# ruotianluo/ImageCaptioning.pytorch

Hardware: NVIDIA H100
Metric: captions/sec at beam=5 seq_len=20 (higher is better)
Workload: dtype f32 (fp32-grade: split-fp16 x3 tensor-core passes, fp32 accumulate)

## Files before the change

imagecaptioning.pytorch_b200/_lib.py:

```python
from __future__ import annotations

import ctypes
import os
from ctypes import POINTER, Structure, c_char_p, c_double, c_float, c_int, c_long, c_longlong, c_ulonglong, c_void_p

PKG = os.path.dirname(os.path.abspath(__file__))
LIB_PATH = os.path.join(PKG, 'libcapb200.so')

MODE_SIMT_FP32, MODE_TC_F16X3, MODE_TC_F16X1 = 0, 1, 2
MODES = {'simt_fp32': MODE_SIMT_FP32, 'tc_f16x3': MODE_TC_F16X3, 'tc_f16x1': MODE_TC_F16X1}
OP_MODES = dict(MODES, skinny_tf32x3=3, skinny_fp32=4, tf32x3_tc=5, tf32x3_tc_dgrad=6, tf32x3_tc_wgrad=7)
FAMILY_UPDOWN, FAMILY_NEWFC, FAMILY_ATT2IN2 = 0, 1, 2
FAMILY_AOA = 3
ENSEMBLE_MAX_MEMBERS = 8
SAMPLE_GREEDY, SAMPLE_MULTINOMIAL, SAMPLE_FORCED, SAMPLE_TEACHER, SAMPLE_TOPK, SAMPLE_TOPP = 0, 1, 2, 3, 4, 5


class ModelCfg(Structure):
    _fields_ = [('family', c_int), ('vocab_size', c_int), ('input_encoding_size', c_int), ('rnn_size', c_int), ('att_hid_size', c_int),
                ('fc_feat_size', c_int), ('att_feat_size', c_int), ('seq_length', c_int), ('numeric_mode', c_int)]


WEIGHT_FIELDS = ['embed', 'fc_embed_w', 'fc_embed_b', 'att_embed_w', 'att_embed_b', 'ctx2att_w', 'ctx2att_b', 'logit_w', 'logit_b',
                 'att_lstm_w_ih', 'att_lstm_w_hh', 'att_lstm_b_ih', 'att_lstm_b_hh', 'lang_lstm_w_ih', 'lang_lstm_w_hh', 'lang_lstm_b_ih',
# ... 107 lines not shown


class MhaWeights(Structure):
    _fields_ = [(f, c_void_p) for f in ('q_w', 'q_b', 'k_w', 'k_b', 'v_w', 'v_b', 'o_w', 'o_b')]


class TfmEncLayer(Structure):
    _fields_ = [('self_attn', MhaWeights)] + [(f, c_void_p) for f in ('w1_w', 'w1_b', 'w2_w', 'w2_b', 'ln0_a', 'ln0_b', 'ln1_a', 'ln1_b')]


class TfmDecLayer(Structure):
    _fields_ = [('self_attn', MhaWeights), ('src_attn', MhaWeights)] + \
               [(f, c_void_p) for f in ('w1_w', 'w1_b', 'w2_w', 'w2_b', 'ln0_a', 'ln0_b', 'ln1_a', 'ln1_b', 'ln2_a', 'ln2_b')]


class TfmWeights(Structure):
    _fields_ = [('att_embed_w', c_void_p), ('att_embed_b', c_void_p), ('enc', TfmEncLayer * TFM_MAX_LAYERS), ('enc_norm_a', c_void_p),
                ('enc_norm_b', c_void_p), ('dec', TfmDecLayer * TFM_MAX_LAYERS), ('dec_norm_a', c_void_p), ('dec_norm_b', c_void_p),
                ('lut', c_void_p), ('pe', c_void_p), ('gen_w', c_void_p), ('gen_b', c_void_p)]


class TfmXeOpts(Structure):
    _fields_ = [('seq_per_img', c_int), ('seed', c_ulonglong), ('label_smoothing', c_float), ('upstream', c_float), ('drop_prob_lm', c_float),
                ('dropout', c_float), ('att_masks', c_void_p), ('keep_rows', c_int), ('row_loss', c_void_p)]


class TfmScstOpts(Structure):
    _fields_ = [('sample_n', c_int), ('temperature', c_float), ('seed', c_ulonglong), ('upstream', c_float), ('baseline', c_int),
                ('drop_prob_lm', c_float), ('dropout', c_float), ('forced_tokens', c_void_p), ('att_masks', c_void_p), ('keep_rows', c_int),
                ('row_loss', c_void_p), ('sampler', POINTER(SamplerOpts)), ('reward_weights', POINTER(RewardWeights))]


class VjpOpts(Structure):
    _fields_ = [('forward_only', c_int), ('dlogprobs', c_void_p), ('greedy', c_int)]


AOA_REFINER_LAYERS = 6


class AoaCfg(Structure):
    _fields_ = [(f, c_int) for f in ('vocab_size', 'input_encoding_size', 'rnn_size', 'heads', 'att_feat_size', 'seq_length', 'numeric_mode')]


class AoaRefinerLayer(Structure):
    _fields_ = [(f, c_void_p) for f in ('q_w', 'q_b', 'k_w', 'k_b', 'v_w', 'v_b', 'aoa_w', 'aoa_b', 'ln_a', 'ln_b')]


class AoaWeights(Structure):
    _fields_ = [('embed', c_void_p), ('att_embed_w', c_void_p), ('att_embed_b', c_void_p), ('refiner', AoaRefinerLayer * AOA_REFINER_LAYERS)] + \
               [(f, c_void_p) for f in ('refiner_norm_a', 'refiner_norm_b', 'ctx2att_w', 'ctx2att_b', 'att_lstm_w_ih', 'att_lstm_w_hh', 'att_lstm_b_ih',
                                        'att_lstm_b_hh', 'attn_norm_a', 'attn_norm_b', 'attn_q_w', 'attn_q_b', 'att2ctx_w', 'att2ctx_b', 'logit_w',
                                        'logit_b')]


class GemmEpilogue(Structure):
    _fields_ = [('bias', c_void_p), ('row_bias', c_void_p), ('ld_row_bias', c_long), ('rows_per_group', c_int), ('residual', c_void_p),
                ('ld_res', c_long), ('relu', c_int), ('C', c_void_p), ('ldc', c_long), ('C_hi', c_void_p), ('C_lo', c_void_p), ('ldcs', c_long),
                ('lstm', c_int), ('H', c_int), ('c_prev', c_void_p), ('ld_cprev', c_long), ('src_row', c_void_p), ('c_out', c_void_p),
                ('ld_cout', c_long), ('gather_bias', c_void_p), ('ld_gb', c_long), ('gather_idx', c_void_p), ('h_f', c_void_p), ('h_hi', c_void_p),
                ('h_lo', c_void_p), ('ld_h', c_long)]


SIGNATURES = {
    'capb200_last_error': (c_char_p, []),
    'capb200_abi_version': (c_int, []),
    'capb200_range_status': (c_int, [c_int]),
    'capb200_linear': (c_int, [c_void_p, c_long, c_void_p, c_long, c_void_p, c_void_p, c_long, c_int, c_int, c_int, c_int, c_int, c_void_p]),
    'capb200_bench_linear': (c_int, [c_void_p, c_void_p, c_void_p, c_void_p, c_int, c_int, c_int, c_int, c_int, c_void_p, c_void_p]),
    'capb200_gemm_tile_n': (c_int, [c_int, c_int]),
    'capb200_gemm_tile_m': (c_int, [c_int, c_int]),
    'capb200_lstm_cell': (c_int, [c_void_p, c_int, c_void_p, c_void_p, c_void_p, c_void_p, c_void_p, c_void_p, c_void_p, c_void_p, c_int, c_int,
                                  c_int, c_void_p]),
    'capb200_additive_attention': (c_int, [c_void_p, c_void_p, c_void_p, c_void_p, c_void_p, c_void_p, c_void_p, c_int, c_int, c_int, c_int, c_int,
                                           c_void_p]),
    'capb200_log_softmax_topk': (c_int, [c_void_p, c_long, c_int, c_int, c_int, c_int, c_void_p, c_void_p, c_void_p]),
    'capb200_vocab_stats_topk': (c_int, [c_void_p, c_long, c_int, c_int, c_int, c_int, c_void_p, c_void_p, c_void_p, c_void_p]),
    'capb200_vocab_select': (c_int, [c_void_p, c_long, c_int, c_int, c_int, c_float, c_float, c_ulonglong, c_ulonglong, c_void_p, c_int, c_void_p,
                                     c_void_p, c_void_p]),
    'capb200_engine_create': (c_void_p, [POINTER(ModelCfg)]),
    'capb200_engine_destroy': (None, [c_void_p]),
    'capb200_engine_bind_weights': (c_int, [c_void_p, POINTER(Weights), c_void_p]),
    'capb200_decode_beam': (c_int, [c_void_p, c_void_p, c_void_p, c_void_p, c_int, c_int, POINTER(BeamOpts), c_void_p, c_void_p, c_void_p, c_void_p,
                                    c_void_p, c_void_p, c_void_p]),
    'capb200_beam_record_logprobs': (c_int, [c_void_p, c_int, c_int, c_void_p, c_void_p]),
    'capb200_decode_beam_diverse': (c_int, [c_void_p, c_void_p, c_void_p, c_void_p, c_int, c_int, POINTER(DiverseOpts), c_void_p, c_void_p, c_void_p,
                                            c_void_p, c_void_p, c_void_p, c_void_p]),
    'capb200_decode_sample': (c_int, [c_void_p, c_void_p, c_void_p, c_void_p, c_int, c_int, POINTER(SampleOpts), c_void_p, c_long, c_void_p, c_void_p,
                                      c_void_p, c_void_p]),
    'capb200_engine_launch_count': (c_long, [c_void_p]),
    'capb200_engine_set_profiling': (c_int, [c_void_p, c_int]),
    'capb200_engine_read_profile': (c_int, [c_void_p, c_int, c_void_p, c_void_p, c_void_p, c_int]),
    'capb200_tfm_create': (c_void_p, [POINTER(TfmCfg)]),
    'capb200_tfm_destroy': (None, [c_void_p]),
    'capb200_tfm_bind_weights': (c_int, [c_void_p, POINTER(TfmWeights), c_void_p]),
    'capb200_tfm_decode_beam': (c_int, [c_void_p, c_void_p, c_void_p, c_int, c_int, POINTER(BeamOpts), c_void_p, c_void_p, c_void_p, c_void_p, c_void_p,
                                        c_void_p, c_void_p]),
    'capb200_tfm_beam_record_logprobs': (c_int, [c_void_p, c_int, c_int, c_void_p, c_void_p]),
    'capb200_tfm_decode_sample': (c_int, [c_void_p, c_void_p, c_void_p, c_int, c_int, POINTER(SampleOpts), c_void_p, c_long, c_void_p, c_void_p, c_void_p,
                                          c_void_p]),
    'capb200_tfm_launch_count': (c_long, [c_void_p]),
    'capb200_aoa_create': (c_void_p, [POINTER(AoaCfg)]),
    'capb200_aoa_destroy': (None, [c_void_p]),
    'capb200_aoa_bind_weights': (c_int, [c_void_p, POINTER(AoaWeights), c_void_p]),
    'capb200_aoa_decode_beam': (c_int, [c_void_p, c_void_p, c_void_p, c_int, c_int, POINTER(BeamOpts), c_void_p, c_void_p, c_void_p, c_void_p, c_void_p,
                                        c_void_p, c_void_p]),
    'capb200_aoa_beam_record_logprobs': (c_int, [c_void_p, c_int, c_int, c_void_p, c_void_p]),
    'capb200_aoa_decode_beam_diverse': (c_int, [c_void_p, c_void_p, c_void_p, c_int, c_int, POINTER(DiverseOpts), c_void_p, c_void_p, c_void_p, c_void_p,
                                                c_void_p, c_void_p, c_void_p]),
    'capb200_aoa_decode_sample': (c_int, [c_void_p, c_void_p, c_void_p, c_int, c_int, POINTER(SampleOpts), c_void_p, c_long, c_void_p, c_void_p, c_void_p,
                                          c_void_p]),
    'capb200_aoa_scst_step': (c_int, [c_void_p, c_void_p, c_int, c_int, POINTER(AoaScstOpts), c_void_p, c_void_p, c_void_p, c_int, POINTER(AoaWeights),
                                      c_void_p, c_void_p, c_void_p, c_void_p, c_void_p, c_void_p]),
    'capb200_aoa_xe_step': (c_int, [c_void_p, c_void_p, c_int, c_int, POINTER(AoaXeOpts), c_void_p, c_void_p, c_int, POINTER(AoaWeights), c_void_p,
                                    c_void_p, c_void_p]),
    'capb200_aoa_launch_count': (c_long, [c_void_p]),
    'capb200_ensemble_create': (c_void_p, []),
    'capb200_ensemble_destroy': (None, [c_void_p]),
    'capb200_ensemble_decode_beam': (c_int, [c_void_p, c_void_p, c_int, c_void_p, c_void_p, c_void_p, c_int, c_int, POINTER(BeamOpts), c_void_p, c_void_p,
                                             c_void_p, c_void_p, c_void_p, c_void_p, c_void_p]),
    'capb200_ensemble_beam_record_logprobs': (c_int, [c_void_p, c_int, c_int, c_void_p, c_void_p]),
    'capb200_ensemble_decode_sample': (c_int, [c_void_p, c_void_p, c_int, c_void_p, c_void_p, c_void_p, c_int, c_int, POINTER(SampleOpts), c_void_p, c_long,
                                               c_void_p, c_void_p, c_void_p, c_void_p]),
    'capb200_ensemble_launch_count': (c_long, [c_void_p]),
    'capb200_updown_scst_step': (c_int, [c_void_p, c_void_p, c_void_p, c_int, c_int, POINTER(ScstOpts), c_void_p, c_void_p, c_void_p, c_int,
                                         POINTER(UpdownGrads), c_void_p, c_void_p, c_void_p, c_void_p, c_void_p, c_void_p]),
    'capb200_att2in2_scst_step': (c_int, [c_void_p, c_void_p, c_void_p, c_int, c_int, POINTER(ScstOpts), c_void_p, c_void_p, c_void_p, c_int,
                                          POINTER(Att2in2Grads), c_void_p, c_void_p, c_void_p, c_void_p, c_void_p, c_void_p]),
    'capb200_att2in2_xe_step': (c_int, [c_void_p, c_void_p, c_void_p, c_int, c_int, POINTER(XeOpts), c_void_p, c_void_p, c_int, POINTER(Att2in2Grads),
                                        c_void_p, c_void_p, c_void_p]),
    'capb200_newfc_scst_step': (c_int, [c_void_p, c_void_p, c_void_p, c_int, c_int, POINTER(ScstOpts), c_void_p, c_void_p, c_void_p, c_int,
                                        POINTER(NewfcGrads), c_void_p, c_void_p, c_void_p, c_void_p, c_void_p, c_void_p]),
    'capb200_newfc_xe_step': (c_int, [c_void_p, c_void_p, c_void_p, c_int, c_int, POINTER(XeOpts), c_void_p, c_void_p, c_int, POINTER(NewfcGrads),
                                      c_void_p, c_void_p, c_void_p]),
    'capb200_dropout_mask': (c_int, [c_void_p, c_long, c_ulonglong, c_int, c_int, c_float, c_void_p]),
    'capb200_mha_forward': (c_int, [c_int, c_int, c_int, c_int, c_int, c_int, c_void_p, c_void_p, c_void_p, c_long, c_void_p, c_long, c_ulonglong, c_int,
                                    c_float, c_void_p, c_long, c_void_p]),
    'capb200_mha_self_backward': (c_int, [c_int, c_int, c_int, c_int, c_int, c_void_p, c_void_p, c_void_p, c_long, c_void_p, c_long, c_ulonglong, c_int,
                                          c_float, c_void_p, c_long, c_void_p, c_void_p, c_void_p, c_long, c_void_p]),
    'capb200_mha_cross_backward': (c_int, [c_int, c_int, c_int, c_int, c_int, c_int, c_int, c_void_p, c_long, c_void_p, c_void_p, c_long, c_ulonglong,
                                           c_int, c_int, c_float, c_void_p, c_void_p, c_long, c_void_p, c_long, c_void_p, c_void_p, c_long, c_void_p]),
    'capb200_mha_causal_forward': (c_int, [c_int, c_int, c_int, c_int, c_int, c_int, c_int, c_void_p, c_void_p, c_void_p, c_long, c_void_p, c_long,
                                           c_ulonglong, c_int, c_float, c_void_p, c_long, c_void_p]),
    'capb200_mha_causal_backward': (c_int, [c_int, c_int, c_int, c_int, c_int, c_void_p, c_void_p, c_void_p, c_long, c_void_p, c_long, c_ulonglong,
                                            c_int, c_float, c_void_p, c_long, c_void_p, c_void_p, c_void_p, c_long, c_void_p]),
    'capb200_tfm_dec_self_attention': (c_int, [c_int, c_int, c_int, c_int, c_int, c_void_p, c_long, c_void_p, c_void_p, c_long, c_long, c_void_p,
                                               c_long, c_void_p, c_long, c_void_p, c_long, c_void_p]),
    'capb200_tfm_xe_step': (c_int, [c_void_p, c_void_p, c_int, c_int, POINTER(TfmXeOpts), c_void_p, c_void_p, c_int, POINTER(TfmWeights), c_void_p, c_void_p,
                                    c_void_p]),
    'capb200_tfm_scst_step': (c_int, [c_void_p, c_void_p, c_int, c_int, POINTER(TfmScstOpts), c_void_p, c_void_p, c_void_p, c_int, POINTER(TfmWeights),
                                      c_void_p, c_void_p, c_void_p, c_void_p, c_void_p, c_void_p]),
    'capb200_tfm_set_grad_events': (c_int, [c_void_p, c_void_p, c_int]),
    'capb200_adam_chunk_elems': (c_int, []),
    'capb200_adam_step': (c_int, [c_void_p, c_void_p, c_void_p, c_int, c_double, c_double, c_double, c_double, c_double, c_long, c_double, c_int, c_void_p]),
    'capb200_engine_set_grad_events': (c_int, [c_void_p, c_void_p, c_int]),
    'capb200_aoa_set_grad_events': (c_int, [c_void_p, c_void_p, c_int]),
    'capb200_cider_table_create': (c_void_p, [c_void_p, c_void_p, c_long, c_double, c_void_p]),
    'capb200_cider_table_destroy': (None, [c_void_p]),
    'capb200_cider_corpus_table_create': (c_void_p, []),
    'capb200_cider_table_reserve': (c_int, [c_void_p, c_long, c_int]),
    'capb200_cider_table_is_corpus': (c_int, [c_void_p]),
    'capb200_cider_scores': (c_int, [c_void_p, c_void_p, c_int, c_int, c_int, c_void_p, c_void_p, c_int, c_void_p, c_void_p, c_void_p]),
    'capb200_bleu4_scores': (c_int, [c_void_p, c_int, c_void_p, c_int, c_int, c_void_p, c_void_p, c_int, c_void_p, c_void_p]),
    'capb200_weighted_reward': (c_int, [c_void_p, POINTER(RewardWeights), c_void_p, c_int, c_void_p, c_int, c_int, c_void_p, c_void_p, c_int, c_void_p,
                                        c_void_p, c_void_p, c_void_p]),
    'capb200_updown_xe_step': (c_int, [c_void_p, c_void_p, c_void_p, c_int, c_int, POINTER(XeOpts), c_void_p, c_void_p, c_int, c_void_p, c_void_p,
                                       c_void_p, c_void_p]),
# ... 68 lines not shown
```

imagecaptioning.pytorch_b200/csrc/beam.cu:

```cuda
#include "../../include/capb200.h"
#include "common.cuh"
#include "kernels.cuh"

namespace capb200 {

namespace {

constexpr int MAXB = 16;

__device__ __forceinline__ double apply_penalty(int kind, float alpha, int length, double p) {
    if (kind == 1) return p / (pow(5.0 + length, (double)alpha) / pow(6.0, (double)alpha));
    if (kind == 2) return p / (double)length;
    return p;
}

__device__ __forceinline__ void select_step(const BeamState& s, int img, int t, int live, int kl, int row0, int hist0, const float* __restrict__ top_val,
                                            const int* __restrict__ top_idx, const int* pen, int n_pen, float lambda, int penalty_kind,
                                            float penalty_alpha, double* __restrict__ done_p) {
    const int lane = threadIdx.x;
    const int b = s.beam, T = s.T;
    const int ncand = live * kl;
    float cv[8];
    int cf[8];
#pragma unroll
    for (int u = 0; u < 8; ++u) {
        const int c = lane + 32 * u;
        cv[u] = -INFINITY;
        cf[u] = 0x7fffffff;
        if (c < ncand) {
            const int pb = c / kl, k = c % kl;
            const long row = (long)row0 + pb;
            const int w = top_idx[row * kl + k];
            float v = top_val[row * kl + k];
            int cnt = 0;
            for (int q = 0; q < n_pen; ++q) cnt += (pen[q] == w);
            if (cnt) v = __fsub_rn(v, __fmul_rn((float)cnt, lambda));
            cv[u] = s.sums[(long)img * b + pb] + v;
            cf[u] = pb * s.V1 + w;
        }
    }
    const int* seq_old = (t & 1) ? s.seq_b : s.seq_a;
    int* seq_new = (t & 1) ? s.seq_a : s.seq_b;
    const int* hist_old = (t & 1) ? s.hist_b : s.hist_a;
    int* hist_new = (t & 1) ? s.hist_a : s.hist_b;

    float my_v = -INFINITY;
    int my_f = 0;
    for (int j = 0; j < b; ++j) {
        float bv = -INFINITY;
        int bf = 0x7fffffff, bu = -1;
#pragma unroll
        for (int u = 0; u < 8; ++u)
            if (cv[u] > bv || (cv[u] == bv && cf[u] < bf)) { bv = cv[u]; bf = cf[u]; bu = u; }
        float wv = bv;
        int wf = bf;
#pragma unroll
        for (int o = 16; o > 0; o >>= 1) {
            const float ov = __shfl_xor_sync(0xffffffffu, wv, o);
            const int of = __shfl_xor_sync(0xffffffffu, wf, o);
            if (ov > wv || (ov == wv && of < wf)) { wv = ov; wf = of; }
        }
        if (bu >= 0 && bf == wf && bv == wv) {
#pragma unroll
            for (int u = 0; u < 8; ++u) if (u == bu) { cv[u] = -INFINITY; cf[u] = 0x7fffffff; }
        }
        if (lane == j) { my_v = wv; my_f = wf; }
    }
    __shared__ int sh_parent[MAXB], sh_word[MAXB], sh_slot[MAXB];
    const bool has = lane < b;
    const int parent = has ? my_f / s.V1 : 0;
    const int word = has ? my_f % s.V1 : 0;
    const bool ended = has && ((word == 0) || (t == T - 1));
    const unsigned em = __ballot_sync(0xffffffffu, ended);
    const int cnt0 = s.done_cnt[img];
    const int slot = cnt0 + __popc(em & ((1u << lane) - 1u));
    if (has) { sh_parent[lane] = parent; sh_word[lane] = word; sh_slot[lane] = ended ? slot : -1; }
    __syncwarp();
    for (int idx = lane; idx < b * t; idx += 32) {
        const int j = idx / t, q = idx - j * t;
        const long dst = ((long)img * b + j) * T, src = ((long)img * b + sh_parent[j]) * T;
        seq_new[dst + q] = seq_old[src + q];
        hist_new[dst + q] = hist_old[src + q];
    }
    if (em != 0u) {
        for (int idx = lane; idx < b * (t + 1); idx += 32) {
            const int j = idx / (t + 1), q = idx - j * (t + 1);
            if (sh_slot[j] < 0) continue;
            const long rec = ((long)img * b * T + sh_slot[j]) * T, src = ((long)img * b + sh_parent[j]) * T;
            s.done_seq[rec + q] = (q < t) ? seq_old[src + q] : sh_word[j];
            s.done_hist[rec + q] = (q < t) ? hist_old[src + q] : hist0 + sh_parent[j];
        }
    }
    if (has) {
        const long dst = ((long)img * b + lane) * T;
        seq_new[dst + t] = word;
        hist_new[dst + t] = hist0 + parent;
        float new_sum = my_v;
        if (ended) {
            const long rec = (long)img * b * T + slot;
            s.done_len[rec] = t + 1;
            s.done_raw[rec] = new_sum;
            done_p[rec] = apply_penalty(penalty_kind, penalty_alpha, t + 1, (double)new_sum);
            new_sum -= 1000.0f;
        }
        s.sums[(long)img * b + lane] = new_sum;
        s.tokens[(long)img * b + lane] = word;
        s.src_row[(long)img * b + lane] = row0 + parent;
    }
    if (lane == 0 && em != 0u) s.done_cnt[img] = cnt0 + __popc(em);
}

__global__ void __launch_bounds__(32) beam_step_kernel(BeamState s, int t, int live, const float* __restrict__ top_val,
                                                       const int* __restrict__ top_idx, int penalty_kind, float penalty_alpha,
                                                       double* __restrict__ done_p) {
    const int img = blockIdx.x;
    select_step(s, img, t, live, s.beam, img * live, img * live, top_val, top_idx, nullptr, 0, 0.f, penalty_kind, penalty_alpha, done_p);
}

__global__ void __launch_bounds__(32) diverse_beam_step_kernel(BeamState s, int G, int t, int k, const float* __restrict__ top_val,
                                                               const int* __restrict__ top_idx, float lambda, int rows_total, int penalty_kind,
                                                               float penalty_alpha, double* __restrict__ done_p) {
    const int i = blockIdx.x, lane = threadIdx.x;
    const int b = s.beam, T = s.T;
    __shared__ int sh_pen[MAXB];
    for (int g = 0; g < G && g <= t; ++g) {
        const int lt = t - g;
        if (lt >= T) continue;
        const int n_pen = g * b;
        __syncwarp();
        if (lane < n_pen) {
            const int pg = lane / b, j = lane - pg * b;
            const int last = min(t - pg, T - 1);
            const int* seq_pg = (last & 1) ? s.seq_a : s.seq_b;
            sh_pen[lane] = seq_pg[((long)(i * G + pg) * b + j) * T + lt];
        }
        __syncwarp();
        const int vimg = i * G + g;
        select_step(s, vimg, lt, lt == 0 ? 1 : b, k, vimg * b, g * rows_total + vimg * b, top_val, top_idx, sh_pen, n_pen, lambda, penalty_kind,
                    penalty_alpha, done_p);
    }
}

__global__ void __launch_bounds__(32) beam_finalize_kernel(BeamState s, int keep, const double* __restrict__ done_p, long long* __restrict__ out_seq,
                                                           int* __restrict__ out_len, float* __restrict__ out_p, float* __restrict__ out_raw,
                                                           int* __restrict__ out_hist) {
    const int img = blockIdx.x, lane = threadIdx.x;
    const int b = s.beam, T = s.T;
    const int cnt = s.done_cnt[img];
    const long base = (long)img * b * T;
    extern __shared__ unsigned char taken[];
    for (int i = lane; i < cnt; i += 32) taken[i] = 0;
    __syncwarp();
    for (int k = 0; k < keep; ++k) {
        double bv = -INFINITY;
        int bi = 0x7fffffff;
        for (int i = lane; i < cnt; i += 32) {
            if (!taken[i]) {
                const double v = done_p[base + i];
                if (v > bv || (v == bv && i < bi)) { bv = v; bi = i; }
            }
        }
#pragma unroll
        for (int o = 16; o > 0; o >>= 1) {
            const double ov = __shfl_xor_sync(0xffffffffu, bv, o);
            const int oi = __shfl_xor_sync(0xffffffffu, bi, o);
            if (ov > bv || (ov == bv && oi < bi)) { bv = ov; bi = oi; }
        }
        const long o = (long)img * keep + k;
        if (bi == 0x7fffffff) {
            if (lane == 0) { out_len[o] = 0; out_p[o] = -INFINITY; out_raw[o] = -INFINITY; }
            for (int q = lane; q < T; q += 32) { out_seq[o * T + q] = 0; out_hist[o * T + q] = -1; }
            continue;
        }
        if (lane == 0) {
            taken[bi] = 1;
            out_len[o] = s.done_len[base + bi];
            out_p[o] = (float)bv;
            out_raw[o] = s.done_raw[base + bi];
        }
        const int len = s.done_len[base + bi];
        for (int q = lane; q < T; q += 32) {
            out_seq[o * T + q] = (q < len) ? (long long)s.done_seq[(base + bi) * T + q] : 0;
            out_hist[o * T + q] = (q < len) ? s.done_hist[(base + bi) * T + q] : -1;
        }
        __syncwarp();
    }
}

__global__ void beam_edit_kernel(int rows, int k_in, int beam, int t, DecodeEdits ed, const int* __restrict__ prev_tokens,
                                 const float* __restrict__ val_in, const int* __restrict__ idx_in, float* __restrict__ val_out, int* __restrict__ idx_out,
                                 int first_beam, int first_group_rows, int first_group) {
    const int r = blockIdx.x * blockDim.x + threadIdx.x;
    if (r >= rows) return;
    if (first_beam > 0 && (r % first_beam) / first_group_rows == first_group) t = 0;
    float v[MAXB];
    int ix[MAXB];
    const int prev = (t > 0 && prev_tokens != nullptr) ? prev_tokens[r] : -1;
    bool prev_bad = false;
    if (t > 0 && ed.n_bad > 0)
        for (int i = 0; i < ed.n_bad; ++i) prev_bad |= (ed.bad[i] == prev);
    for (int k = 0; k < k_in; ++k) {
        float x = val_in[(long)r * k_in + k];
        const int w = idx_in[(long)r * k_in + k];
        if (ed.constraint && t > 0 && w == prev) x = -INFINITY;
        if (prev_bad && w == 0) x = -INFINITY;
        if (w == ed.unk_col) x -= 1000.0f;
        v[k] = x;
        ix[k] = w;
    }
    for (int j = 0; j < beam; ++j) {
        int best = j;
        for (int k = j + 1; k < k_in; ++k)
            if (v[k] > v[best] || (v[k] == v[best] && ix[k] < ix[best])) best = k;
        const float tv = v[j]; v[j] = v[best]; v[best] = tv;
        const int ti = ix[j]; ix[j] = ix[best]; ix[best] = ti;
        val_out[(long)r * beam + j] = v[j];
        idx_out[(long)r * beam + j] = ix[j];
    }
}

__global__ void scale_rows_kernel(float* __restrict__ x, long ld, int rows, int cols, float f, int skip_beam, int skip_group_rows, int skip_group) {
    const long total = (long)rows * cols;
// ... 16 lines not shown
        return;
    }
    auto apply_edits = [&]() {
        if (seqs == nullptr || !ed.any()) return;
        __syncthreads();
        if (threadIdx.x == 0) {
            const int prev = sidx > 0 ? (int)seqs[item - 1] : -1;
            if (ed.unk_col >= 0 && ed.unk_col < V1) d[ed.unk_col] -= 1000.0f;
            if (ed.constraint && prev >= 0 && prev < V1) d[prev] = -INFINITY;
            bool prev_bad = false;
            for (int i = 0; i < ed.n_bad; ++i) prev_bad |= (sidx > 0 && ed.bad[i] == prev);
            if (prev_bad) d[0] = -INFINITY;
        }
    };
    const float* src = slab + (long)sidx * step_stride + (long)row * ld_slab;
    if (stats != nullptr) {
        const float2 st = stats[(long)sidx * stats_stride + row];
        const float mx = st.x, lsum = st.y;
        const float m2 = (mx - mx) - lsum, l2 = lsum;
        const bool twice = sidx > 0;
        const bool vec4 = ((V1 & 3) == 0) && ((ld_slab & 3) == 0) && ((step_stride & 3) == 0) && ((reinterpret_cast<uintptr_t>(slab) & 15) == 0) &&
                          ((reinterpret_cast<uintptr_t>(dst) & 15) == 0);
        if (vec4) {
            const float4* s4 = reinterpret_cast<const float4*>(src);
            float4* d4 = reinterpret_cast<float4*>(d);
            for (int v = threadIdx.x; v < V1 / 4; v += blockDim.x) {
                const float4 x = __ldg(s4 + v);
                float4 o;
                o.x = (x.x - mx) - lsum; o.y = (x.y - mx) - lsum; o.z = (x.z - mx) - lsum; o.w = (x.w - mx) - lsum;
                if (twice) { o.x = (o.x - m2) - l2; o.y = (o.y - m2) - l2; o.z = (o.z - m2) - l2; o.w = (o.w - m2) - l2; }
                d4[v] = o;
            }
        } else {
            for (int v = threadIdx.x; v < V1; v += blockDim.x) {
                const float lp = (src[v] - mx) - lsum;
                d[v] = twice ? (lp - m2) - l2 : lp;
            }
        }
        apply_edits();
        return;
    }
    const bool vec = ((V1 & 3) == 0) && ((ld_slab & 3) == 0) && ((step_stride & 3) == 0) && ((reinterpret_cast<uintptr_t>(slab) & 15) == 0) &&
                     ((reinterpret_cast<uintptr_t>(dst) & 15) == 0);
    if (vec) {
        const float4* s4 = reinterpret_cast<const float4*>(src);
        float4* d4 = reinterpret_cast<float4*>(d);
        for (int v = threadIdx.x; v < V1 / 4; v += blockDim.x) d4[v] = __ldg(s4 + v);
    } else {
        for (int v = threadIdx.x; v < V1; v += blockDim.x) d[v] = src[v];
    }
    apply_edits();
}

}

int beam_edit_launch(int rows, int k_in, int beam, int t, const DecodeEdits& ed, const int* prev_tokens, const float* val_in, const int* idx_in,
                     float* val_out, int* idx_out, cudaStream_t stream, int first_beam, int first_group_rows, int first_group) {
    CAPB_REQUIRE(k_in >= beam && k_in <= MAXB, "beam_size + number of active decode edits must be <= 16");
    if (rows <= 0) return 0;
    beam_edit_kernel<<<cdiv(rows, 128), 128, 0, stream>>>(rows, k_in, beam, t, ed, prev_tokens, val_in, idx_in, val_out, idx_out, first_beam,
                                                          first_group_rows, first_group);
    CAPB_CHECK_CUDA(cudaGetLastError());
    return 0;
}

int scale_rows_launch(float* x, long ld, int rows, int cols, float factor, cudaStream_t stream, int skip_beam, int skip_group_rows, int skip_group) {
    if (rows <= 0 || cols <= 0) return 0;
    long blocks = ((long)rows * cols + 255) / 256;
    if (blocks > sm_count() * 16) blocks = sm_count() * 16;
    scale_rows_kernel<<<(int)blocks, 256, 0, stream>>>(x, ld, rows, cols, factor, skip_beam, skip_group_rows, skip_group);
    CAPB_CHECK_CUDA(cudaGetLastError());
    return 0;
}

int beam_step_launch(const BeamState& s, int t, int live, const float* top_val, const int* top_idx, int penalty_kind, float penalty_alpha,
                     cudaStream_t stream) {
    CAPB_REQUIRE(s.beam >= 1 && s.beam <= MAXB, "beam size 1..16");
    CAPB_REQUIRE(s.beam * s.T <= MAXB * CAPB200_MAX_SEQ_LENGTH, "beam*T record capacity (16 x CAPB200_MAX_SEQ_LENGTH)");
    beam_step_kernel<<<s.B, 32, 0, stream>>>(s, t, live, top_val, top_idx, penalty_kind, penalty_alpha, s.done_p);
    CAPB_CHECK_CUDA(cudaGetLastError());
    return 0;
}

int diverse_beam_step_launch(const BeamState& s, int G, int t, int k, const float* top_val, const int* top_idx, float lambda, int rows_total,
                             int penalty_kind, float penalty_alpha, cudaStream_t stream) {
    CAPB_REQUIRE(G >= 2 && s.beam >= 1 && G * s.beam <= MAXB, "group_size * beams per group must be in 2..16");
    CAPB_REQUIRE(k >= s.beam && k <= MAXB && s.beam * k <= 256, "candidate list width");
    CAPB_REQUIRE(s.beam * s.T <= MAXB * CAPB200_MAX_SEQ_LENGTH, "beam*T record capacity (16 x CAPB200_MAX_SEQ_LENGTH)");
    CAPB_REQUIRE(lambda >= 0.f, "diversity_lambda must be >= 0 (the candidate lists rely on the penalty only lowering values)");
    diverse_beam_step_kernel<<<s.B / G, 32, 0, stream>>>(s, G, t, k, top_val, top_idx, lambda, rows_total, penalty_kind, penalty_alpha, s.done_p);
    CAPB_CHECK_CUDA(cudaGetLastError());
    return 0;
}

int beam_finalize_launch(const BeamState& s, int keep, long long* out_seq, int* out_len, float* out_p, float* out_raw, int* out_hist,
                         cudaStream_t stream) {
    CAPB_REQUIRE(keep >= 1 && keep <= s.beam, "keep must be in 1..beam");
    beam_finalize_kernel<<<s.B, 32, (size_t)s.beam * s.T, stream>>>(s, keep, s.done_p, out_seq, out_len, out_p, out_raw, out_hist);
    CAPB_CHECK_CUDA(cudaGetLastError());
    return 0;
}

int gather_logprob_rows_launch(const float* slab, long step_stride, long ld_slab, const int* hist, int nseq, int T, int V1, float* dst,
                               const float2* stats, long stats_stride, cudaStream_t stream, const long long* seqs, const DecodeEdits* ed) {
    if (nseq <= 0) return 0;
    gather_rows_kernel<<<nseq * T, 256, 0, stream>>>(slab, step_stride, ld_slab, hist, T, V1, dst, stats, stats_stride, seqs, ed ? *ed : DecodeEdits());
    CAPB_CHECK_CUDA(cudaGetLastError());
    return 0;
}

}
```

imagecaptioning.pytorch_b200/csrc/engine.cu:

```cuda
#include <map>
#include <mutex>
#include <vector>

#include "../../include/capb200.h"
#include "common.cuh"
#include "kernels.cuh"
#include "engine_common.cuh"
#include "train_common.cuh"

namespace capb200 {

static thread_local std::string g_last_error;
void set_error(const std::string& msg) { g_last_error = msg; }
const char* last_error_cstr() { return g_last_error.c_str(); }

__global__ void capb_fill_int_kernel(int* p, int n, int v) {
    const int i = blockIdx.x * blockDim.x + threadIdx.x;
    if (i < n) p[i] = v;
}
__global__ void capb_load_token_column_kernel(const long long* src, long ld, int col, int n, int* dst) {
    const int i = blockIdx.x * blockDim.x + threadIdx.x;
    if (i < n) dst[i] = (int)src[(long)i * ld + col];
}
__global__ void capb_store_token_column_kernel(const int* src, int n, long long* dst, long ld, int col) {
// ... 218 lines not shown
    }
    return gemm_tc_plan_launch(e->plans[id], &g.epi, g.M, st);
}

int run_gemm(capb200_engine* e, int id, GemmProblem& g, int plan_rows, cudaStream_t st) {
    if (!e->profiling) return run_gemm_inner(e, id, g, plan_rows, st);
    if (e->ev_used + 2 > e->ev_pool.size()) {
        for (int i = 0; i < 64; ++i) {
            cudaEvent_t ev;
            CAPB_CHECK_CUDA(cudaEventCreate(&ev));
            e->ev_pool.push_back(ev);
        }
    }
    double k_total = 0;
    for (int s = 0; s < g.nseg; ++s) k_total += g.seg[s].K;
    CAPB_CHECK_CUDA(cudaEventRecord(e->ev_pool[e->ev_used], st));
    const int rc = run_gemm_inner(e, id, g, plan_rows, st);
    CAPB_CHECK_CUDA(cudaEventRecord(e->ev_pool[e->ev_used + 1], st));
    e->ev_used += 2;
    e->ev_ids.push_back(id);
    e->ev_flops.push_back(2.0 * g.M * g.N * k_total);
    return rc;
}

int prepare(capb200_engine* e, const float* fc, const float* att, const float* mask, int B, int R, cudaStream_t st) {
    CAPB_NVTX("capb200 prepare_feature (fc_embed, att_embed, ctx2att)");
    const int H = e->H, E = e->E, A = e->A;
    const bool updown = e->cfg.family == CAPB200_FAMILY_UPDOWN;
    const capb200_weights& w = e->w;
    ActView fc_in;  fc_in.f = const_cast<float*>(fc);  fc_in.ld = e->cfg.fc_feat_size;
    if (e->tc && e->cfg.family != CAPB200_FAMILY_ATT2IN2) {
        e->launches++;
        if (split_planes_launch(fc, e->cfg.fc_feat_size, B, e->cfg.fc_feat_size, e->in_fc.hi, e->in_fc.lo, e->in_fc.ld, st)) return 1;
    }
    if (e->cfg.family != CAPB200_FAMILY_ATT2IN2) {
        GemmProblem g;
        g.M = B; g.N = updown ? H : E; g.nseg = 1;
        g.seg[0] = seg_of(fc_in, w.fc_embed_w, e->cfg.fc_feat_size, e->p_fc, e->cfg.fc_feat_size);
        g.seg[0].A_hi = e->in_fc.hi; g.seg[0].A_lo = e->in_fc.lo; g.seg[0].lda_h = e->in_fc.ld;
        g.epi.bias = w.fc_embed_b; g.epi.relu = updown ? 1 : 0;
        g.epi.C = e->fc_e.v.f; g.epi.ldc = e->fc_e.v.ld; g.epi.C_hi = e->fc_e.v.hi; g.epi.C_lo = e->fc_e.v.lo; g.epi.ldcs = e->fc_e.v.ld;
        if (run_gemm(e, G_FC, g, e->capB, st)) return 1;
    }
    if (!attends(e)) return 0;
    ActView att_in; att_in.f = const_cast<float*>(att); att_in.ld = e->cfg.att_feat_size;
    if (e->tc) {
        e->launches++;
        if (split_planes_launch(att, e->cfg.att_feat_size, B * R, e->cfg.att_feat_size, e->in_att.hi, e->in_att.lo, e->in_att.ld, st)) return 1;
    }
    {
        GemmProblem g;
        g.M = B * R; g.N = H; g.nseg = 1;
        g.seg[0] = seg_of(att_in, w.att_embed_w, e->cfg.att_feat_size, e->p_attw, e->cfg.att_feat_size);
        g.seg[0].A_hi = e->in_att.hi; g.seg[0].A_lo = e->in_att.lo; g.seg[0].lda_h = e->in_att.ld;
        g.epi.bias = w.att_embed_b; g.epi.relu = 1;
        g.epi.C = e->att_e.v.f; g.epi.ldc = e->att_e.v.ld; g.epi.C_hi = e->att_e.v.hi; g.epi.C_lo = e->att_e.v.lo; g.epi.ldcs = e->att_e.v.ld;
        if (run_gemm(e, G_ATT, g, e->capB * e->capR, st)) return 1;
    }
    if (mask != nullptr) {
        e->launches++;
        if (mask_rows_launch(e->att_e.v, B, R, H, mask, R, st)) return 1;
    }
    {
        GemmProblem g;
        g.M = B * R; g.N = A; g.nseg = 1;
        g.seg[0] = seg_of(e->att_e.v, w.ctx2att_w, H, e->p_ctx, H);
        g.epi.bias = w.ctx2att_b;
        g.epi.C = e->p_att.v.f; g.epi.ldc = e->p_att.v.ld;
        if (run_gemm(e, G_CTX, g, e->capB * e->capR, st)) return 1;
    }
    if (!updown) return 0;
    {
        GemmProblem g;
        g.M = B; g.N = 4 * H; g.nseg = 1;
        g.seg[0] = seg_of(e->fc_e.v, w.att_lstm_w_ih + H, E + 2 * H, e->p_a_ih_fc, H);
        g.epi.bias = e->tc ? e->bsum_att_il : e->bsum_att;
        g.epi.C = e->g_fc.v.f; g.epi.ldc = e->g_fc.v.ld;
        if (run_gemm(e, G_GFC, g, e->capB, st)) return 1;
    }
    return 0;
}

int core_step(capb200_engine* e, int rows, int rpi, const int* tokens, const int* src_row, float* logits, long ld_logits, int n_images, int R,
              const float* mask, cudaStream_t st) {
    const int H = e->H, E = e->E, A = e->A, V1 = e->V1;
    const capb200_weights& w = e->w;
    if (e->cfg.family == CAPB200_FAMILY_UPDOWN) {
        StateCopy s0, s1;
        s0.src = e->h0_out.v.f; s0.ld_src = e->h0_out.v.ld; s0.dst = e->h0_in.v;
        s1.src = e->h1_out.v.f; s1.ld_src = e->h1_out.v.ld; s1.dst = e->h1_in.v;
        const bool xg = e->use_xgate;
        e->launches++;
        if (state_gather_embed_launch(rows, tokens, src_row, w.embed, E, xg ? 0 : E, 1, e->xt.v, H, 2, s0, s1, st)) return 1;
        const int cur = e->core_cur, nxt = cur ^ 1;
        {
            GemmProblem g;
            g.M = rows; g.N = 4 * H;
            g.seg[0] = seg_of(e->h1_in.v, w.att_lstm_w_ih, E + 2 * H, e->p_a_ih_h, H);
            g.seg[1] = seg_of(e->h0_in.v, w.att_lstm_w_hh, H, e->p_a_hh, H);
            g.nseg = 2;
            if (!xg) { g.seg[2] = seg_of(e->xt.v, w.att_lstm_w_ih + 2 * H, E + 2 * H, e->p_a_ih_x, E); g.nseg = 3; }
            g.epi.row_bias = e->g_fc.v.f; g.epi.ld_row_bias = e->g_fc.v.ld; g.epi.rows_per_group = rpi;
            if (e->tc) {
                g.epi.lstm = 1; g.epi.H = H;
                g.epi.c_prev = e->c0[cur]; g.epi.ld_cprev = e->ld_c; g.epi.src_row = src_row;
                g.epi.c_out = e->c0[nxt]; g.epi.ld_cout = e->ld_c;
                g.epi.gather_bias = xg ? e->xgate : nullptr; g.epi.ld_gb = e->ld_xgate; g.epi.gather_idx = tokens;
                g.epi.h_f = e->h0_out.v.f; g.epi.h_hi = e->h0_out.v.hi; g.epi.h_lo = e->h0_out.v.lo; g.epi.ld_h = e->h0_out.v.ld;
            } else {
                g.epi.C = e->gates.v.f; g.epi.ldc = e->gates.v.ld;
            }
            if (run_gemm(e, G_LSTM1, g, e->capRows, st)) return 1;
        }
        if (!e->tc) {
            e->launches++;
            if (lstm_pointwise_launch(rows, H, e->gates.v.f, e->gates.v.ld, src_row, e->c0[cur], e->ld_c, e->c0[nxt], e->ld_c, e->h0_out.v,
                                      xg ? e->xgate : nullptr, e->ld_xgate, tokens, st)) return 1;
        }
        {
            GemmProblem g;
            g.M = rows; g.N = A; g.nseg = 1;
            g.seg[0] = seg_of(e->h0_out.v, w.h2att_w, H, e->p_h2att, H);
            g.epi.bias = w.h2att_b;
            g.epi.C = e->att_h.v.f; g.epi.ldc = e->att_h.v.ld;
            if (run_gemm(e, G_H2ATT, g, e->capRows, st)) return 1;
        }
        e->launches += 2;
        if (additive_attention_launch(n_images, rpi, R, A, H, e->att_h.v.f, e->att_h.v.ld, e->p_att.v.f, e->p_att.v.ld, e->att_e.v.f, e->att_e.v.ld,
                                      mask, R, w.alpha_w, w.alpha_b, e->att_score, e->att_res.v, st)) return 1;
        {
            GemmProblem g;
            g.M = rows; g.N = 4 * H; g.nseg = 3;
            g.seg[0] = seg_of(e->att_res.v, w.lang_lstm_w_ih, 2 * H, e->p_l_ih_a, H);
            g.seg[1] = seg_of(e->h0_out.v, w.lang_lstm_w_ih + H, 2 * H, e->p_l_ih_h, H);
            g.seg[2] = seg_of(e->h1_in.v, w.lang_lstm_w_hh, H, e->p_l_hh, H);
            if (e->tc) {
                g.epi.bias = e->bsum_lang_il;
                g.epi.lstm = 1; g.epi.H = H;
                g.epi.c_prev = e->c1[cur]; g.epi.ld_cprev = e->ld_c; g.epi.src_row = src_row;
                g.epi.c_out = e->c1[nxt]; g.epi.ld_cout = e->ld_c;
                g.epi.h_f = e->h1_out.v.f; g.epi.h_hi = e->h1_out.v.hi; g.epi.h_lo = e->h1_out.v.lo; g.epi.ld_h = e->h1_out.v.ld;
            } else {
                g.epi.bias = e->bsum_lang;
                g.epi.C = e->gates.v.f; g.epi.ldc = e->gates.v.ld;
            }
            if (run_gemm(e, G_LSTM2, g, e->capRows, st)) return 1;
        }
        if (!e->tc) {
            e->launches++;
            if (lstm_pointwise_launch(rows, H, e->gates.v.f, e->gates.v.ld, src_row, e->c1[cur], e->ld_c, e->c1[nxt], e->ld_c, e->h1_out.v,
                                      nullptr, 0, nullptr, st)) return 1;
        }
        e->core_cur = nxt;
        {
            GemmProblem g;
            g.M = rows; g.N = V1; g.nseg = 1;
            g.seg[0] = seg_of(e->h1_out.v, w.logit_w, H, e->p_logit, H);
            g.epi.bias = w.logit_b;
            g.epi.C = logits; g.epi.ldc = ld_logits;
            if (run_gemm(e, G_LOGIT, g, e->capRows, st)) return 1;
        }
        return 0;
    }
    if (e->cfg.family == CAPB200_FAMILY_ATT2IN2) {
        StateCopy s0, s1;
        s0.src = e->h0_out.v.f; s0.ld_src = e->h0_out.v.ld; s0.dst = e->h0_in.v;
        e->launches++;
        if (state_gather_embed_launch(rows, tokens, src_row, w.embed, E, E, 1, e->xt.v, H, 1, s0, s1, st)) return 1;
        const int cur = e->core_cur, nxt = cur ^ 1;
        {
            GemmProblem g;
            g.M = rows; g.N = A; g.nseg = 1;
            g.seg[0] = seg_of(e->h0_in.v, w.h2att_w, H, e->p_h2att, H);
            g.epi.bias = w.h2att_b;
            g.epi.C = e->att_h.v.f; g.epi.ldc = e->att_h.v.ld;
            if (run_gemm(e, G_H2ATT, g, e->capRows, st)) return 1;
// ... 16 lines not shown
            g.seg[0] = seg_of(e->att_res.v, w.a2c_w, H, e->p_a2c, H);
            g.epi.residual = e->gates.v.f + 3 * H; g.epi.ld_res = e->gates.v.ld;
            g.epi.C = e->gates.v.f + 3 * H; g.epi.ldc = e->gates.v.ld;
            if (run_gemm(e, G_A2C, g, e->capRows, st)) return 1;
        }
        e->launches++;
        if (maxout_pointwise_launch(rows, H, e->gates.v.f, e->gates.v.ld, src_row, e->c0[cur], e->ld_c, e->c0[nxt], e->ld_c, e->h0_out.v, st)) return 1;
        e->core_cur = nxt;
        GemmProblem g;
        g.M = rows; g.N = V1; g.nseg = 1;
        g.seg[0] = seg_of(e->h0_out.v, w.logit_w, H, e->p_logit, H);
        g.epi.bias = w.logit_b;
        g.epi.C = logits; g.epi.ldc = ld_logits;
        return run_gemm(e, G_LOGIT, g, e->capRows, st);
    }
    const bool fresh = (src_row == e->d.neg1);
    for (int pass = fresh ? 0 : 1; pass < 2; ++pass) {
        StateCopy s0, s1;
        s0.src = e->h0_out.v.f; s0.ld_src = e->h0_out.v.ld; s0.dst = e->h0_in.v;
        const int* srcs = (pass == 0) ? e->d.neg1 : (fresh ? nullptr : src_row);
        e->launches++;
        if (pass == 0) {
            if (state_gather_embed_launch(rows, e->img_of_row, srcs, e->fc_e.v.f, e->fc_e.v.ld, E, 0, e->xt.v, H, 1, s0, s1, st)) return 1;
        } else {
            if (state_gather_embed_launch(rows, tokens, srcs, w.embed, E, E, 0, e->xt.v, H, 1, s0, s1, st)) return 1;
        }
        const int cur = e->core_cur, nxt = cur ^ 1;
        GemmProblem g;
        g.M = rows; g.N = 5 * H; g.nseg = 2;
        g.seg[0] = seg_of(e->xt.v, w.i2h_w, E, e->p_i2h, E);
        g.seg[1] = seg_of(e->h0_in.v, w.h2h_w, H, e->p_h2h, H);
        g.epi.bias = e->bsum_core;
        g.epi.C = e->gates.v.f; g.epi.ldc = e->gates.v.ld;
        if (run_gemm(e, G_CORE, g, e->capRows, st)) return 1;
        e->launches++;
        if (maxout_pointwise_launch(rows, H, e->gates.v.f, e->gates.v.ld, srcs, e->c0[cur], e->ld_c, e->c0[nxt], e->ld_c, e->h0_out.v, st)) return 1;
        e->core_cur = nxt;
    }
    GemmProblem g;
    g.M = rows; g.N = V1; g.nseg = 1;
    g.seg[0] = seg_of(e->h0_out.v, w.logit_w, H, e->p_logit, H);
    g.epi.bias = w.logit_b;
    g.epi.C = logits; g.epi.ldc = ld_logits;
    return run_gemm(e, G_LOGIT, g, e->capRows, st);
}

int check_ready(capb200_engine* e) {
    CAPB_REQUIRE(e != nullptr, "null engine");
    CAPB_REQUIRE(e->bound, "capb200_engine_bind_weights has not been called");
    CAPB_CHECK_RANGE();
    return 0;
}

}

namespace capb200 {

int lstm_member_info(capb200_engine* e, MemberInfo* m) {
    if (check_ready(e)) return 1;
    m->family = e->cfg.family;
    m->V1 = e->V1; m->T = e->T;
    m->attends = attends(e);
    m->graph_ok = !e->profiling;
    m->ws = e->ws; m->wblock = e->wblock;
    m->fresh = e->d.neg1;
    m->launches = &e->launches;
    return 0;
}

int lstm_decode_workspace(capb200_engine* e, int B, int rows, int R, int beam, int rows_per_image, cudaStream_t st) {
    if (ensure_workspace(e, B, rows, R, beam, st)) return 1;
    if (!attends(e)) { iota_div_kernel<<<cdiv(rows, 256), 256, 0, st>>>(e->img_of_row, rows, rows_per_image); e->launches++; }
    return 0;
}

int lstm_decode_prepare(capb200_engine* e, const float* fc, const float* att, const float* mask, int B, int R, cudaStream_t st) {
    if (prepare(e, fc, att, mask, B, R, st)) return 1;
    e->core_cur = 0;
    return 0;
}

int lstm_decode_core(capb200_engine* e, int rows, int rpi, const int* tokens, const int* src_row, float* logits, long ld, int B, int R,
                     const float* mask, cudaStream_t st) {
    return core_step(e, rows, rpi, tokens, src_row, logits, ld, B, R, mask, st);
}

}

extern "C" {

const char* capb200_last_error(void) { return g_last_error.c_str(); }
int capb200_abi_version(void) { return CAPB200_ABI_VERSION; }
int capb200_range_status(int reset) { return range_flag_read(reset); }

capb200_engine* capb200_engine_create(const capb200_model_cfg* cfg) {
    if (cfg == nullptr) { set_error("null cfg"); return nullptr; }
    if (cfg->family != CAPB200_FAMILY_UPDOWN && cfg->family != CAPB200_FAMILY_NEWFC && cfg->family != CAPB200_FAMILY_ATT2IN2) {
        set_error("unknown model family");
        return nullptr;
    }
    if (cfg->numeric_mode < 0 || cfg->numeric_mode > 2) { set_error("unknown numeric mode"); return nullptr; }
    if (cfg->seq_length < 1 || cfg->seq_length > CAPB200_MAX_SEQ_LENGTH) { set_error("seq_length must be in 1..256 (CAPB200_MAX_SEQ_LENGTH)"); return nullptr; }
    int ndev = 0;
    if (cudaGetDeviceCount(&ndev) != cudaSuccess || ndev == 0) {
        set_error("no CUDA device: the capb200 engine has no CPU fallback");
        return nullptr;
    }
    capb200_engine* e = new capb200_engine();
    e->cfg = *cfg;
    e->V1 = cfg->vocab_size + 1;
    e->E = cfg->input_encoding_size;
    e->H = cfg->rnn_size;
    e->A = cfg->att_hid_size;
    e->T = cfg->seq_length;
    e->mode = cfg->numeric_mode;
    e->tc = cfg->numeric_mode != CAPB200_MODE_SIMT_FP32;
    return e;
}

void capb200_engine_destroy(capb200_engine* e) {
    if (e == nullptr) return;
    destroy_plans(e);
    for (cudaEvent_t ev : e->ev_pool) cudaEventDestroy(ev);
    cudaFree(e->wblock);
    cudaFree(e->ws);
    e->d.release();
    cudaFree(e->tape);
    e->sg.destroy();
    tf32_context_destroy(e->tf32);
    if (e->ev_gfork) cudaEventDestroy(e->ev_gfork);
    if (e->ev_gjoin) cudaEventDestroy(e->ev_gjoin);
    if (e->side) cudaStreamDestroy(e->side);
    delete e;
}

long capb200_engine_launch_count(const capb200_engine* e) { return e ? e->launches : 0; }

int capb200_engine_set_profiling(capb200_engine* e, int enable) {
    CAPB_REQUIRE(e != nullptr, "null engine");
    e->profiling = enable != 0;
    return 0;
}

int capb200_engine_read_profile(capb200_engine* e, int reset, double* ms, double* flops, long* calls, int n) {
    CAPB_REQUIRE(e != nullptr && n >= G_REPORTED, "need room for 9 GEMM ids");
    CAPB_CHECK_CUDA(cudaDeviceSynchronize());
    for (size_t i = 0; i < e->ev_ids.size(); ++i) {
        float t = 0.f;
        CAPB_CHECK_CUDA(cudaEventElapsedTime(&t, e->ev_pool[2 * i], e->ev_pool[2 * i + 1]));
        e->prof_ms[e->ev_ids[i]] += t;
        e->prof_flops[e->ev_ids[i]] += e->ev_flops[i];
        e->prof_calls[e->ev_ids[i]] += 1;
    }
    e->ev_ids.clear();
    e->ev_flops.clear();
    e->ev_used = 0;
    e->prof_ms[G_CORE] += e->prof_ms[G_A2C]; e->prof_flops[G_CORE] += e->prof_flops[G_A2C]; e->prof_calls[G_CORE] += e->prof_calls[G_A2C];
    e->prof_ms[G_A2C] = 0; e->prof_flops[G_A2C] = 0; e->prof_calls[G_A2C] = 0;
    for (int i = 0; i < G_REPORTED; ++i) {
        if (ms) ms[i] = e->prof_ms[i];
        if (flops) flops[i] = e->prof_flops[i];
        if (calls) calls[i] = e->prof_calls[i];
        if (reset) { e->prof_ms[i] = 0; e->prof_flops[i] = 0; e->prof_calls[i] = 0; }
    }
    return 0;
}

// ... 37 lines not shown
        if (att2in2) {
            add_vec_kernel<<<cdiv(2 * H, 256), 256, 0, st>>>(e->bsum_core + 3 * H, w->a2c_b, e->bsum_core + 3 * H, 2 * H);
            e->launches += 1;
        }
    }
    CAPB_CHECK_CUDA(cudaGetLastError());
    if (e->tc) {
        int rc = pack(e, w->logit_w, H, V1, H, e->p_logit, st);
        if (updown) {
            rc |= pack(e, w->fc_embed_w, e->cfg.fc_feat_size, H, e->cfg.fc_feat_size, e->p_fc, st);
            rc |= pack(e, w->att_embed_w, e->cfg.att_feat_size, H, e->cfg.att_feat_size, e->p_attw, st);
            rc |= pack(e, w->ctx2att_w, H, A, H, e->p_ctx, st);
            rc |= pack_gates(e, w->att_lstm_w_ih, E + 2 * H, H, H, e->p_a_ih_h, st);
            rc |= pack_gates(e, w->att_lstm_w_ih + H, E + 2 * H, H, H, e->p_a_ih_fc, st);
            rc |= pack_gates(e, w->att_lstm_w_ih + 2 * H, E + 2 * H, H, E, e->p_a_ih_x, st);
            rc |= pack_gates(e, w->att_lstm_w_hh, H, H, H, e->p_a_hh, st);
            rc |= pack_gates(e, w->lang_lstm_w_ih, 2 * H, H, H, e->p_l_ih_a, st);
            rc |= pack_gates(e, w->lang_lstm_w_ih + H, 2 * H, H, H, e->p_l_ih_h, st);
            rc |= pack_gates(e, w->lang_lstm_w_hh, H, H, H, e->p_l_hh, st);
            rc |= pack(e, w->h2att_w, H, A, H, e->p_h2att, st);
        } else if (att2in2) {
            rc |= pack(e, w->att_embed_w, e->cfg.att_feat_size, H, e->cfg.att_feat_size, e->p_attw, st);
            rc |= pack(e, w->ctx2att_w, H, A, H, e->p_ctx, st);
            rc |= pack(e, w->h2att_w, H, A, H, e->p_h2att, st);
            rc |= pack(e, w->i2h_w, E, 5 * H, E, e->p_i2h, st);
            rc |= pack(e, w->h2h_w, H, 5 * H, H, e->p_h2h, st);
            rc |= pack(e, w->a2c_w, H, 2 * H, H, e->p_a2c, st);
        } else {
            rc |= pack(e, w->fc_embed_w, e->cfg.fc_feat_size, E, e->cfg.fc_feat_size, e->p_fc, st);
            rc |= pack(e, w->i2h_w, E, 5 * H, E, e->p_i2h, st);
            rc |= pack(e, w->h2h_w, H, 5 * H, H, e->p_h2h, st);
        }
        if (rc) return 1;
    }
    if (updown) {
        const long n = (long)V1 * E;
        const long ldE = round_up(E, 8);
        char* tmp = nullptr;
        const size_t tmp_bytes = (size_t)V1 * ldE * (sizeof(float) + (e->tc ? 2 * sizeof(__half) : 0)) + 1024;
        CAPB_CHECK_CUDA(cudaMallocAsync(&tmp, tmp_bytes, st));
        ActView ev;
        ev.ld = ldE;
        ev.f = reinterpret_cast<float*>(tmp);
        if (e->tc) {
            ev.hi = reinterpret_cast<__half*>(tmp + (size_t)V1 * ldE * sizeof(float));
            ev.lo = ev.hi + (size_t)V1 * ldE;
        }
        int rc = 0;
        if (ldE == E) {
            rc = relu_copy_launch(w->embed, n, ev, st);
        } else {
            CAPB_CHECK_CUDA(cudaMemsetAsync(tmp, 0, tmp_bytes, st));
            for (int v = 0; v < V1 && !rc; ++v) {
                ActView rv = ev;
                rv.f += (long)v * ldE; if (rv.hi) { rv.hi += (long)v * ldE; rv.lo += (long)v * ldE; }
                rc = relu_copy_launch(w->embed + (long)v * E, E, rv, st);
            }
        }
        GemmProblem g;
        g.M = V1; g.N = 4 * H; g.nseg = 1;
        g.seg[0] = seg_of(ev, w->att_lstm_w_ih + 2 * H, E + 2 * H, e->p_a_ih_x, E);
        g.epi.C = e->xgate; g.epi.ldc = e->ld_xgate;
        if (!rc) {
            if (!e->tc) {
                rc = gemm_simt_launch(g, st);
            } else {
                GemmTcPlan* plan = gemm_tc_plan_create(g, e->mode == CAPB200_MODE_TC_F16X3 ? 3 : 1);
                rc = plan ? gemm_tc_plan_launch(plan, nullptr, 0, st) : 1;
                if (plan) gemm_tc_plan_destroy(plan);
            }
        }
        e->launches += 2;
        cudaFreeAsync(tmp, st);
        if (rc) return 1;
    }
    if (e->tc && !e->bound) {
        CAPB_CHECK_CUDA(cudaStreamSynchronize(st));
        CAPB_CHECK_RANGE();
    }
    e->bound = true;
    return 0;
}

int capb200_decode_beam(capb200_engine* e, const float* fc, const float* att, const float* mask, int B, int R, const capb200_beam_opts* opts,
                        long long* seq, float* seq_logprobs, long long* done_seq, int* done_len, float* done_p, float* done_raw, void* stream) {
    if (check_ready(e)) return 1;
    cudaStream_t st = static_cast<cudaStream_t>(stream);
    CAPB_REQUIRE(opts != nullptr && (fc != nullptr || e->cfg.family == CAPB200_FAMILY_ATT2IN2) && seq != nullptr, "null argument");
    const int beam = opts->beam_size, keep = opts->sample_n;
    CAPB_REQUIRE(beam >= 1 && beam <= 16 && beam <= e->V1, "beam_size must be in 1..16 and <= V+1");
    CAPB_REQUIRE(keep == 1 || keep == beam, "sample_n must be 1 or beam_size (AttModel.py:223)");
    CAPB_REQUIRE(B >= 1, "empty batch");
    const bool attn = attends(e);
    if (attn) CAPB_REQUIRE(att != nullptr && R >= 1, "attention features required");
    if (!attn) R = 1;
    const int T = e->T, V1 = e->V1;
    const int rows = B * beam;
    if (lstm_decode_workspace(e, B, rows, R, beam, 1, st)) return 1;
    if (lstm_decode_prepare(e, fc, att, mask, B, R, st)) return 1;
    auto core = [&](int nrows, int live, const int* tokens, const int* src_row, int , float* logits, long ld) {
        return lstm_decode_core(e, nrows, live, tokens, src_row, logits, ld, B, R, mask, st);
    };
    return beam_decode_driver(e->d, V1, T, B, beam, keep, opts->penalty_kind, opts->penalty_alpha, seq, seq_logprobs, done_seq, done_len, done_p,
                              done_raw, core, &e->launches, st, e->profiling ? 0ull : loop_graph_key(e->ws, e->wblock, mask, R, (int)e->cfg.family),
                              to_edits(opts->edits), opts->temperature);
}

int capb200_decode_beam_diverse(capb200_engine* e, const float* fc, const float* att, const float* mask, int B, int R, const capb200_diverse_opts* opts,
                                long long* seq, float* seq_logprobs, long long* done_seq, int* done_len, float* done_p, float* done_raw, void* stream) {
    if (check_ready(e)) return 1;
    cudaStream_t st = static_cast<cudaStream_t>(stream);
    CAPB_REQUIRE(opts != nullptr && (fc != nullptr || e->cfg.family == CAPB200_FAMILY_ATT2IN2) && seq != nullptr, "null argument");
    CAPB_REQUIRE(attends(e), "diverse beam search runs on UpDown and Att2in2 (NewFC's fresh-state pass is chosen per call, not per row)");
    if (opts->group_size == 1) return capb200_decode_beam(e, fc, att, mask, B, R, &opts->base, seq, seq_logprobs, done_seq, done_len, done_p, done_raw, stream);
    const int beam = opts->base.beam_size;
    CAPB_REQUIRE(beam >= 2 && beam <= 16 && beam <= e->V1, "beam_size must be in 2..16 and <= V+1");
    CAPB_REQUIRE(B >= 1, "empty batch");
    CAPB_REQUIRE(att != nullptr && R >= 1, "attention features required");
    const int rows = B * beam;
    if (lstm_decode_workspace(e, B, rows, R, beam, 1, st)) return 1;
    if (lstm_decode_prepare(e, fc, att, mask, B, R, st)) return 1;
    auto core = [&](int nrows, int rpi, const int* tokens, const int* src_row, int , float* logits, long ld) {
        return lstm_decode_core(e, nrows, rpi, tokens, src_row, logits, ld, B, R, mask, st);
    };
    return diverse_beam_decode_driver(e->d, e->V1, e->T, B, beam, opts->group_size, opts->diversity_lambda, opts->base.sample_n, opts->base.penalty_kind,
                                      opts->base.penalty_alpha, seq, seq_logprobs, done_seq, done_len, done_p, done_raw, core, &e->launches, st,
                                      e->profiling ? 0ull : loop_graph_key(e->ws, e->wblock, mask, R, (int)e->cfg.family), to_edits(opts->base.edits),
                                      opts->base.temperature);
}

int capb200_beam_record_logprobs(capb200_engine* e, int image, int rank, float* dst, void* stream) {
    if (check_ready(e)) return 1;
    return beam_record_logprobs(e->d, e->V1, e->T, image, rank, dst, static_cast<cudaStream_t>(stream));
}

int capb200_decode_sample(capb200_engine* e, const float* fc, const float* att, const float* mask, int B, int R, const capb200_sample_opts* opts,
                          const long long* tokens_in, long ld_tok, long long* seq, float* seq_logprobs, float* picked, void* stream) {
    if (check_ready(e)) return 1;
    cudaStream_t st = static_cast<cudaStream_t>(stream);
    CAPB_REQUIRE(opts != nullptr && (fc != nullptr || e->cfg.family == CAPB200_FAMILY_ATT2IN2) && seq_logprobs != nullptr, "null argument");
    const int n = opts->sample_n;
    CAPB_REQUIRE(n >= 1 && B >= 1, "empty batch");
    const bool attn = attends(e);
    if (attn) CAPB_REQUIRE(att != nullptr && R >= 1, "attention features required");
    if (!attn) R = 1;
    const int method = opts->method;
    CAPB_REQUIRE(method >= 0 && method <= 5, "unknown sampling method");
    if (method == CAPB200_SAMPLE_FORCED || method == CAPB200_SAMPLE_TEACHER) CAPB_REQUIRE(tokens_in != nullptr && ld_tok >= 1, "token matrix required");
    if (method != CAPB200_SAMPLE_TEACHER) CAPB_REQUIRE(seq != nullptr, "seq output required");
    if (method == CAPB200_SAMPLE_MULTINOMIAL || method >= CAPB200_SAMPLE_TOPK) CAPB_REQUIRE(opts->temperature > 0.f, "temperature must be positive");
    const int T = e->T, V1 = e->V1;
    const int rows = B * n;
    const int steps = (method == CAPB200_SAMPLE_TEACHER) ? opts->steps : T;
    const long t_out = (method == CAPB200_SAMPLE_TEACHER) ? ld_tok : T;
    CAPB_REQUIRE(steps >= 0 && steps <= t_out, "steps out of range");
    if (lstm_decode_workspace(e, B, rows, R, 1, n, st)) return 1;
    if (lstm_decode_prepare(e, fc, att, mask, B, R, st)) return 1;
    auto core = [&](int nrows, int , const int* tokens, const int* src_row, int , float* logits, long ld) {
        return lstm_decode_core(e, nrows, n, tokens, src_row, logits, ld, B, R, mask, st);
    };
    return sample_decode_driver(e->d, V1, T, rows, method, opts->temperature, opts->seed, steps, tokens_in, ld_tok, seq, seq_logprobs, picked, core,
                                &e->launches, st, to_edits(opts->edits), opts->top);
}

int capb200_linear(const float* x, long ldx, const float* w, long ldw, const float* b, float* y, long ldy, int M, int N, int K, int relu, int mode,
                   void* stream) {
    cudaStream_t st = static_cast<cudaStream_t>(stream);
    CAPB_REQUIRE(x && w && y && M > 0 && N > 0 && K > 0, "bad argument");
    GemmProblem g;
    g.M = M; g.N = N; g.nseg = 1;
    g.seg[0].A = x; g.seg[0].lda = ldx; g.seg[0].W = w; g.seg[0].ldw = ldw; g.seg[0].K = K;
    g.epi.bias = b; g.epi.relu = relu; g.epi.C = y; g.epi.ldc = ldy;
    if (mode == CAPB200_MODE_SIMT_FP32) return gemm_simt_launch(g, st);
    if (mode == CAPB200_MODE_SKINNY_TF32X3 || mode == CAPB200_MODE_SKINNY_FP32) {
        CAPB_REQUIRE(!relu, "the skinny GEMM has no relu epilogue");
        const size_t cap = (size_t)4 << 20;
        float* part = nullptr;
        CAPB_CHECK_CUDA(cudaMallocAsync(&part, cap * sizeof(float), st));
        const int tb = 1;
        const int rc = gemm_skinny_launch(M, N, 1, &x, &ldx, &w, &ldw, &K, &tb, y, ldy, b, nullptr, 0, 1, 0, part, cap, mode == CAPB200_MODE_SKINNY_TF32X3, st);
        cudaFreeAsync(part, st);
        return rc;
    }
    if (mode == CAPB200_MODE_TF32X3_TC || mode == CAPB200_MODE_TF32X3_TC_DGRAD || mode == CAPB200_MODE_TF32X3_TC_WGRAD) {
        CAPB_REQUIRE(!relu, "the tf32 GEMM has no relu epilogue");
        Tf32Context* ctx = tf32_context_create();
        Skinny sk{nullptr, 0, 1, st};
        sk.ctx = ctx;
// ... 903 lines not shown
```

imagecaptioning.pytorch_b200/csrc/engine_common.cuh:

```cuda
#pragma once
#include <cstdio>
#include <cstdlib>
#include <cstring>

#include "../../include/capb200.h"
#include "common.cuh"
#include "kernels.cuh"
#include "nvtx.cuh"

struct capb200_cider_table {
    capb200::CiderTable* t = nullptr;
};

namespace capb200 {

struct Planes {
    __half* hi = nullptr;
    __half* lo = nullptr;
    long ld = 0;
};

struct Arena {
    char* base = nullptr;
    size_t off = 0;
// ... 7 lines not shown
};

struct Act {
    ActView v;
    void carve(Arena& a, long rows, long cols, bool planes) {
        v.ld = round_up(cols, 64);
        v.f = a.take<float>(rows * v.ld);
        if (planes) {
            v.hi = a.take<__half>(rows * v.ld);
            v.lo = a.take<__half>(rows * v.ld);
        } else {
            v.hi = v.lo = nullptr;
        }
    }
};

inline DecodeEdits to_edits(const capb200_decode_edits& c) {
    DecodeEdits e;
    e.constraint = c.decoding_constraint;
    e.unk_col = c.unk_col;
    e.n_bad = (c.bad_endings != nullptr && c.n_bad_endings > 0) ? c.n_bad_endings : 0;
    e.bad = c.bad_endings;
    e.trigrams = c.block_trigrams;
    e.trigram_rows = c.trigram_rows;
    return e;
}

inline Planes carve_planes(Arena& a, long rows, long cols) {
    Planes p;
    p.ld = round_up(cols, 64);
    p.hi = a.take<__half>(rows * p.ld);
    p.lo = a.take<__half>(rows * p.ld);
    return p;
}


inline GemmSeg seg_of(const ActView& a, const float* w, long ldw, const Planes& wp, int K) {
    GemmSeg s;
    s.A = a.f; s.lda = a.ld; s.W = w; s.ldw = ldw;
    s.A_hi = a.hi; s.A_lo = a.lo; s.lda_h = a.ld;
    s.W_hi = wp.hi; s.W_lo = wp.lo; s.ldw_h = wp.ld;
    s.K = K;
    return s;
}


inline int run_gemm_mode(int mode, GemmTcPlan** plan, GemmProblem& g, int plan_rows, cudaStream_t st) {
    if (mode == 0) return gemm_simt_launch(g, st);
    if (*plan == nullptr) {
        GemmProblem planned = g;
        planned.M = plan_rows;
        *plan = gemm_tc_plan_create(planned, mode == 1 ? 3 : 1);
        if (*plan == nullptr) return 1;
    }
    return gemm_tc_plan_launch(*plan, &g.epi, g.M, st);
}


struct DecodeBuffers {
    int *tokens = nullptr, *src_row = nullptr, *neg1 = nullptr, *unfinished = nullptr, *forced = nullptr;
    float* top_val = nullptr;
    int* top_idx = nullptr;
    float* top_val_e = nullptr;
    int* top_idx_e = nullptr;
    float2* slab_stats = nullptr;
    BeamState bs;
    long long* rec_seq = nullptr;
    int *rec_len = nullptr, *rec_hist = nullptr, *out_hist = nullptr, *tmp_len = nullptr;
    float *rec_p = nullptr, *rec_raw = nullptr, *tmp_p = nullptr, *tmp_raw = nullptr;
    float* slab = nullptr;
    size_t slab_bytes = 0;
    float2* dbs_stats = nullptr;
    size_t dbs_stats_bytes = 0;
    int* dbs_done_cnt = nullptr;
    size_t dbs_done_bytes = 0;
    const float2* last_stats = nullptr;
    long slab_step_stride = 0;
    int last_B = 0, last_beam = 0;
    DecodeEdits last_edits;
    cudaGraphExec_t loop_exec = nullptr;
    unsigned long long loop_key[8] = {0, 0, 0, 0, 0, 0, 0, 0}, seen_key[8] = {0, 0, 0, 0, 0, 0, 0, 0};
    long loop_launches = 0;
    bool graph_broken = false;

    void release() {
        if (loop_exec) cudaGraphExecDestroy(loop_exec);
        loop_exec = nullptr;
        cudaFree(slab);
        cudaFree(dbs_stats);
        cudaFree(dbs_done_cnt);
        slab = nullptr; dbs_stats = nullptr; dbs_done_cnt = nullptr;
    }

    void carve(Arena& a, int B, int rows, int beam, int T) {
        tokens = a.take<int>(rows);
        src_row = a.take<int>(rows);
        neg1 = a.take<int>(rows);
        unfinished = a.take<int>(rows);
        forced = a.take<int>(rows);
        top_val = a.take<float>((long)rows * 16);
        top_idx = a.take<int>((long)rows * 16);
        top_val_e = a.take<float>((long)rows * 16);
        top_idx_e = a.take<int>((long)rows * 16);
        slab_stats = a.take<float2>((long)rows * T);
        const long rec = (long)B * beam * T;
        bs.sums = a.take<float>((long)B * beam);
        bs.seq_a = a.take<int>(rec);
        bs.seq_b = a.take<int>(rec);
        bs.hist_a = a.take<int>(rec);
        bs.hist_b = a.take<int>(rec);
        bs.done_cnt = a.take<int>(B);
        bs.done_seq = a.take<int>(rec * T);
        bs.done_hist = a.take<int>(rec * T);
        bs.done_len = a.take<int>(rec);
        bs.done_p = a.take<double>(rec);
        bs.done_raw = a.take<float>(rec);
        bs.tokens = tokens;
        bs.src_row = src_row;
        rec_seq = a.take<long long>(rec);
        rec_hist = a.take<int>(rec);
        out_hist = a.take<int>(rec);
        rec_len = a.take<int>((long)B * beam);
        rec_p = a.take<float>((long)B * beam);
        rec_raw = a.take<float>((long)B * beam);
        tmp_len = a.take<int>((long)B * beam);
        tmp_p = a.take<float>((long)B * beam);
        tmp_raw = a.take<float>((long)B * beam);
    }
};

__global__ void capb_fill_int_kernel(int* p, int n, int v);
__global__ void capb_load_token_column_kernel(const long long* src, long ld, int col, int n, int* dst);
int fill_int_launch(int* p, int n, int v, cudaStream_t st);
int load_token_column_launch(const long long* src, long ld, int col, int n, int* dst, cudaStream_t st);
int store_token_column_launch(const int* src, int n, long long* dst, long ld, int col, cudaStream_t st);

inline const int* beam_ancestors(const BeamState& s, int t) { return ((t - 1) & 1) ? s.hist_a : s.hist_b; }

inline unsigned long long loop_graph_key(const void* ws, const void* wblock, const void* mask, int R, int family) {
    unsigned long long h = 1469598103934665603ull;
    auto mix = [&](unsigned long long v) { h ^= v; h *= 1099511628211ull; };
    mix(reinterpret_cast<uintptr_t>(ws)); mix(reinterpret_cast<uintptr_t>(wblock)); mix(reinterpret_cast<uintptr_t>(mask));
    mix((unsigned long long)R); mix((unsigned long long)family + 17);
    return h | 1ull;
}

inline int grow_buffer(void** p, size_t* bytes, size_t need, cudaStream_t st) {
    if (need <= *bytes) return 0;
    CAPB_CHECK_CUDA(cudaStreamSynchronize(st));
    if (*p) CAPB_CHECK_CUDA(cudaFree(*p));
    *p = nullptr;
    *bytes = 0;
    const cudaError_t e = cudaMalloc(p, need);
    if (e != cudaSuccess) {
        (void)cudaGetLastError();
        *p = nullptr;
        set_error("cannot allocate " + std::to_string(need >> 20) + " MB of device workspace (" + cudaGetErrorString(e) +
                  "); its size grows with batch, length and V + 1: DESIGN.md, 'Vocabularies above 51 199 words'");
        return 1;
    }
    *bytes = need;
    return 0;
}

template <class Loop>
int run_beam_loop(DecodeBuffers& d, const unsigned long long (&key)[8], bool use_graph, long* launches, cudaStream_t st, Loop run_loop) {
    static const bool graphs_off = getenv("CAPB200_NO_GRAPH") != nullptr;
    const bool debug = getenv("CAPB200_GRAPH_DEBUG") != nullptr;
    const bool try_graph = use_graph && !graphs_off && !d.graph_broken;
    if (try_graph && d.loop_exec != nullptr && memcmp(key, d.loop_key, sizeof(key)) == 0) {
        CAPB_CHECK_CUDA(cudaGraphLaunch(d.loop_exec, st));
        *launches += d.loop_launches;
        if (debug) fprintf(stderr, "capb200: beam loop replayed from its CUDA graph\n");
    } else if (try_graph && memcmp(key, d.seen_key, sizeof(key)) == 0) {
        if (d.loop_exec != nullptr) { cudaGraphExecDestroy(d.loop_exec); d.loop_exec = nullptr; }
        const long l0 = *launches;
        cudaGraph_t graph = nullptr;
        bool ok = cudaStreamBeginCapture(st, cudaStreamCaptureModeThreadLocal) == cudaSuccess;
        const int rc = ok ? run_loop() : 1;
        if (ok) ok = cudaStreamEndCapture(st, &graph) == cudaSuccess && graph != nullptr && rc == 0;
        if (ok) ok = cudaGraphInstantiate(&d.loop_exec, graph, 0) == cudaSuccess;
        if (graph != nullptr) cudaGraphDestroy(graph);
        if (!ok) {
            (void)cudaGetLastError();
            d.loop_exec = nullptr;
            d.graph_broken = true;
            *launches = l0;
            if (run_loop()) return 1;
        } else {
            d.loop_launches = *launches - l0;
            memcpy(d.loop_key, key, sizeof(key));
            CAPB_CHECK_CUDA(cudaGraphLaunch(d.loop_exec, st));
            if (debug) fprintf(stderr, "capb200: beam loop captured into a CUDA graph (%ld launches)\n", d.loop_launches);
        }
    } else {
        memcpy(d.seen_key, key, sizeof(key));
        if (run_loop()) return 1;
    }
    return 0;
}

template <class CoreFn>
int beam_decode_driver(DecodeBuffers& d, int V1, int T, int B, int beam, int keep, int penalty_kind, float penalty_alpha, long long* seq,
                       float* seq_logprobs, long long* done_seq, int* done_len, float* done_p, float* done_raw, CoreFn core, long* launches,
                       cudaStream_t st, unsigned long long graph_key = 0, const DecodeEdits& ed = DecodeEdits(), float temperature = 1.0f) {
    const int rows = B * beam;
    const bool edits = ed.any();
    const int k_in = beam + ed.kinds();
    CAPB_REQUIRE(!ed.trigrams, "block_trigrams applies to _sample only (AttModel.py:306)");
    CAPB_REQUIRE(k_in <= 16, "beam_size + number of active decode edits (decoding_constraint, remove_bad_endings, UNK suppression) must be <= 16");
    if (temperature == 0.f) temperature = 1.0f;
    CAPB_REQUIRE(temperature > 0.f, "temperature must be positive");
    if (grow_buffer(reinterpret_cast<void**>(&d.slab), &d.slab_bytes, (size_t)T * rows * V1 * sizeof(float), st)) return 1;
    d.slab_step_stride = (long)rows * V1;
    d.last_B = B;
    d.last_beam = beam;
    BeamState s = d.bs;
    s.B = B; s.beam = beam; s.T = T; s.V1 = V1;
    auto run_loop = [&]() -> int {
        CAPB_NVTX("capb200 beam loop (T steps: core, vocab stats, beam step)");
        CAPB_CHECK_CUDA(cudaMemsetAsync(s.sums, 0, sizeof(float) * B * beam, st));
        CAPB_CHECK_CUDA(cudaMemsetAsync(s.done_cnt, 0, sizeof(int) * B, st));
        CAPB_CHECK_CUDA(cudaMemsetAsync(d.tokens, 0, sizeof(int) * rows, st));
        for (int t = 0; t < T; ++t) {
            const int live = (t == 0) ? 1 : beam;
            const int nrows = B * live;
            float* logits = d.slab + (long)t * d.slab_step_stride;
            if (core(nrows, live, d.tokens, t == 0 ? d.neg1 : d.src_row, t, logits, (long)V1)) return 1;
            if (t > 0 && temperature != 1.0f) {
                if (scale_rows_launch(logits, V1, nrows, V1, 1.0f / temperature, st)) return 1;
                *launches += 1;
            }
            VocabStepArgs va;
            va.rows = nrows; va.V1 = V1; va.logits = logits; va.ld = V1;
            va.twice = (t > 0) ? 1 : 0;
            va.topk = edits ? k_in : beam; va.top_val = d.top_val; va.top_idx = d.top_idx;
            va.stats = d.slab_stats + (long)t * rows;
            if (vocab_step_launch(va, st)) return 1;
            const float* tv = d.top_val;
            const int* ti = d.top_idx;
            if (edits) {
                if (beam_edit_launch(nrows, k_in, beam, t, ed, d.tokens, d.top_val, d.top_idx, d.top_val_e, d.top_idx_e, st)) return 1;
                tv = d.top_val_e; ti = d.top_idx_e;
                *launches += 1;
            }
            if (beam_step_launch(s, t, live, tv, ti, penalty_kind, penalty_alpha, st)) return 1;
            *launches += 2;
        }
        return 0;
    };
    unsigned long long key[8] = {graph_key, (unsigned long long)B, (unsigned long long)beam, (unsigned long long)T, (unsigned long long)V1,
                                 (unsigned long long)penalty_kind, 0ull, (unsigned long long)reinterpret_cast<uintptr_t>(d.slab)};
    memcpy(&key[6], &penalty_alpha, sizeof(float));
    memcpy(reinterpret_cast<char*>(&key[6]) + 4, &temperature, sizeof(float));
    key[5] ^= ((unsigned long long)(ed.constraint & 1) << 8) ^ ((unsigned long long)(unsigned)(ed.unk_col + 1) << 16) ^ ((unsigned long long)ed.n_bad << 48);
    key[0] ^= (unsigned long long)reinterpret_cast<uintptr_t>(ed.bad) * 0x9E3779B97F4A7C15ull;
    d.last_edits = ed;
    d.last_stats = d.slab_stats;
    if (run_beam_loop(d, key, graph_key != 0, launches, st, run_loop)) return 1;
    CAPB_NVTX("capb200 beam finalize + log-prob rows");
    if (beam_finalize_launch(s, beam, d.rec_seq, d.rec_len, d.rec_p, d.rec_raw, d.rec_hist, st)) return 1;
    *launches += 1;
    if (keep == beam) {
        CAPB_CHECK_CUDA(cudaMemcpyAsync(seq, d.rec_seq, sizeof(long long) * B * beam * T, cudaMemcpyDeviceToDevice, st));
        if (seq_logprobs) {
            *launches += 1;
            if (gather_logprob_rows_launch(d.slab, d.slab_step_stride, V1, d.rec_hist, B * beam, T, V1, seq_logprobs, d.slab_stats, rows, st, d.rec_seq, &ed)) return 1;
        }
    } else {
        *launches += 1;
        if (beam_finalize_launch(s, 1, seq, d.tmp_len, d.tmp_p, d.tmp_raw, d.out_hist, st)) return 1;
        if (seq_logprobs) {
            *launches += 1;
            if (gather_logprob_rows_launch(d.slab, d.slab_step_stride, V1, d.out_hist, B, T, V1, seq_logprobs, d.slab_stats, rows, st, seq, &ed)) return 1;
        }
    }
    if (done_seq) CAPB_CHECK_CUDA(cudaMemcpyAsync(done_seq, d.rec_seq, sizeof(long long) * B * beam * T, cudaMemcpyDeviceToDevice, st));
    if (done_len) CAPB_CHECK_CUDA(cudaMemcpyAsync(done_len, d.rec_len, sizeof(int) * B * beam, cudaMemcpyDeviceToDevice, st));
    if (done_p) CAPB_CHECK_CUDA(cudaMemcpyAsync(done_p, d.rec_p, sizeof(float) * B * beam, cudaMemcpyDeviceToDevice, st));
    if (done_raw) CAPB_CHECK_CUDA(cudaMemcpyAsync(done_raw, d.rec_raw, sizeof(float) * B * beam, cudaMemcpyDeviceToDevice, st));
    return 0;
}

template <class CoreFn>
int diverse_beam_decode_driver(DecodeBuffers& d, int V1, int T, int B, int beam, int G, float lambda, int keep, int penalty_kind, float penalty_alpha,
                               long long* seq, float* seq_logprobs, long long* done_seq, int* done_len, float* done_p, float* done_raw, CoreFn core,
                               long* launches, cudaStream_t st, unsigned long long graph_key, const DecodeEdits& ed, float temperature) {
    CAPB_REQUIRE(G >= 2 && beam % G == 0, "diverse beam search needs group_size >= 2 dividing beam_size");
    CAPB_REQUIRE(lambda >= 0.f, "diversity_lambda must be >= 0");
    const int bdash = beam / G, rows = B * beam, steps = T + G - 1;
    CAPB_REQUIRE(keep == 1 || keep == bdash, "sample_n must be 1 or beam_size / group_size (AttModel.py:223)");
    const bool edits = ed.any();
    const int k_in = beam + ed.kinds();
    CAPB_REQUIRE(!ed.trigrams, "block_trigrams applies to _sample only (AttModel.py:306)");
    CAPB_REQUIRE(k_in <= 16, "beam_size + number of active decode edits (decoding_constraint, remove_bad_endings, UNK suppression) must be <= 16");
    if (temperature == 0.f) temperature = 1.0f;
    CAPB_REQUIRE(temperature > 0.f, "temperature must be positive");
    if (grow_buffer(reinterpret_cast<void**>(&d.slab), &d.slab_bytes, (size_t)steps * rows * V1 * sizeof(float), st)) return 1;
    if (grow_buffer(reinterpret_cast<void**>(&d.dbs_stats), &d.dbs_stats_bytes, (size_t)steps * rows * sizeof(float2), st)) return 1;
    if (grow_buffer(reinterpret_cast<void**>(&d.dbs_done_cnt), &d.dbs_done_bytes, (size_t)B * G * sizeof(int), st)) return 1;
    d.slab_step_stride = (long)rows * V1;
    d.last_B = B;
    d.last_beam = beam;
    d.last_edits = ed;
    d.last_stats = d.dbs_stats;
    BeamState s = d.bs;
    s.B = B * G; s.beam = bdash; s.T = T; s.V1 = V1;
    s.done_cnt = d.dbs_done_cnt;
    auto run_loop = [&]() -> int {
        CAPB_NVTX("capb200 diverse beam loop (T+G-1 steps: core, vocab stats, group steps)");
        CAPB_CHECK_CUDA(cudaMemsetAsync(s.sums, 0, sizeof(float) * rows, st));
        CAPB_CHECK_CUDA(cudaMemsetAsync(s.done_cnt, 0, sizeof(int) * B * G, st));
        CAPB_CHECK_CUDA(cudaMemsetAsync(d.tokens, 0, sizeof(int) * rows, st));
        CAPB_CHECK_CUDA(cudaMemsetAsync(d.src_row, 0xff, sizeof(int) * rows, st));
        for (int t = 0; t < steps; ++t) {
            float* logits = d.slab + (long)t * d.slab_step_stride;
            if (core(rows, beam, d.tokens, d.src_row, t, logits, (long)V1)) return 1;
            if (t > 0 && temperature != 1.0f) {
                if (scale_rows_launch(logits, V1, rows, V1, 1.0f / temperature, st, beam, bdash, t)) return 1;
                *launches += 1;
            }
            VocabStepArgs va;
            va.rows = rows; va.V1 = V1; va.logits = logits; va.ld = V1;
            va.twice = (t > 0) ? 1 : 0;
            va.first_beam = beam; va.first_group_rows = bdash; va.first_group = t;
            va.topk = edits ? k_in : beam; va.top_val = d.top_val; va.top_idx = d.top_idx;
            va.stats = d.dbs_stats + (long)t * rows;
            if (vocab_step_launch(va, st)) return 1;
            const float* tv = d.top_val;
            const int* ti = d.top_idx;
            if (edits) {
                if (beam_edit_launch(rows, k_in, beam, t, ed, d.tokens, d.top_val, d.top_idx, d.top_val_e, d.top_idx_e, st, beam, bdash, t)) return 1;
                tv = d.top_val_e; ti = d.top_idx_e;
                *launches += 1;
            }
            if (diverse_beam_step_launch(s, G, t, beam, tv, ti, lambda, rows, penalty_kind, penalty_alpha, st)) return 1;
            *launches += 2;
        }
// ... 252 lines not shown
```

imagecaptioning.pytorch_b200/csrc/kernels.cuh:

```cuda
#pragma once
#include "common.cuh"

namespace capb200 {

struct ActView {
    float* f = nullptr;
    __half* hi = nullptr;
    __half* lo = nullptr;
    long ld = 0;
};

struct StateCopy {
    const float* src = nullptr;
    long ld_src = 0;
    ActView dst;
};

int state_gather_embed_launch(int rows, const int* tokens, const int* src_row, const float* emb, long ld_emb, int E, int relu,
                              ActView xt, int H, int nstate, StateCopy sc0, StateCopy sc1, cudaStream_t stream);
int lstm_pointwise_launch(int rows, int H, const float* gates, long ld_g, const int* src_row, const float* c_prev, long ld_cp,
                          float* c_out, long ld_co, ActView h_out, const float* gather_bias, long ld_gb, const int* gather_idx,
                          cudaStream_t stream);
int relu_copy_launch(const float* x, long n, ActView out_flat, cudaStream_t stream);
int lstm_ln_launch(int rows, int H, const float* gates, long ld_g, const float* c_prev, long ld_cp, float* c_out, long ld_co, float* h_out, long ld_h,
                   const float* ln_a, const float* ln_b, float eps, float* ln_out, long ld_ln, cudaStream_t stream);
int maxout_pointwise_launch(int rows, int H, const float* sums, long ld_s, const int* src_row, const float* c_prev, long ld_cp,
                            float* c_out, long ld_co, ActView h_out, cudaStream_t stream);
int additive_attention_launch(int n_images, int rpi, int R, int A, int H, const float* att_h, long ld_ah, const float* p_att, long ld_pa,
                              const float* att, long ld_at, const float* mask, long ld_mask, const float* alpha_w, const float* alpha_b,
                              float* score_scratch , ActView out, cudaStream_t stream, float* alpha_out = nullptr );
int mask_rows_launch(ActView x, int n_images, int R, int cols, const float* mask, long ld_mask, cudaStream_t stream);
int ss_select_launch(int rows, int V1, const float* prev_logp, long ld, const long long* labels, long ld_labels, int col, unsigned long long seed, float prob,
                     int* tok_out, cudaStream_t stream);

struct DecodeEdits {
    int constraint = 0;
    int unk_col = -1;
    int n_bad = 0;
    const int* bad = nullptr;
    int trigrams = 0;
    int trigram_rows = 0;
    __host__ __device__ bool any() const { return constraint != 0 || unk_col >= 0 || n_bad > 0 || trigrams != 0; }
    __host__ __device__ int kinds() const { return (constraint ? 1 : 0) + (unk_col >= 0 ? 1 : 0) + (n_bad > 0 ? 1 : 0); }
};

struct VocabStepArgs {
    int rows = 0;
    int V1 = 0;
    float* logits = nullptr;
    long ld = 0;
    int twice = 0;
    float2* stats = nullptr;
    int topk = 0;
    float* top_val = nullptr;
    int* top_idx = nullptr;
    int select = 0;
    float top = 0.f;
    DecodeEdits edits;
    const int* prev_tokens = nullptr;
    float temperature = 1.0f;
    unsigned long long seed = 0;
    unsigned long long step = 0;
    const int* forced = nullptr;
    int* unfinished = nullptr;
    int first_step = 0;
    int* tokens_out = nullptr;
    long long* seq_out = nullptr;
    long ld_seq = 0;
    int t = 0;
    float* picked_lp = nullptr;
    long ld_picked = 1;
    int first_beam = 0, first_group_rows = 1, first_group = -1;
    __host__ __device__ int row_twice(int r) const {
        return twice && !(first_beam > 0 && (r % first_beam) / first_group_rows == first_group);
    }
};
int vocab_step_launch(const VocabStepArgs& a, cudaStream_t stream);
int beam_edit_launch(int rows, int k_in, int beam, int t, const DecodeEdits& ed, const int* prev_tokens, const float* val_in, const int* idx_in,
                     float* val_out, int* idx_out, cudaStream_t stream, int first_beam = 0, int first_group_rows = 1, int first_group = -1);
int scale_rows_launch(float* x, long ld, int rows, int cols, float factor, cudaStream_t stream, int skip_beam = 0, int skip_group_rows = 1,
                      int skip_group = -1);

struct BeamState {
    int B = 0, beam = 0, T = 0, V1 = 0;
    float* sums = nullptr;
    int* seq_a = nullptr;
    int* seq_b = nullptr;
    int* hist_a = nullptr;
    int* hist_b = nullptr;
    int* done_cnt = nullptr;
    int* done_seq = nullptr;
    int* done_hist = nullptr;
    int* done_len = nullptr;
    double* done_p = nullptr;
    float* done_raw = nullptr;
    int* tokens = nullptr;
    int* src_row = nullptr;
};
int beam_step_launch(const BeamState& s, int t, int live, const float* top_val, const int* top_idx, int penalty_kind, float penalty_alpha,
                     cudaStream_t stream);
int diverse_beam_step_launch(const BeamState& s, int G, int t, int k, const float* top_val, const int* top_idx, float lambda, int rows_total,
                             int penalty_kind, float penalty_alpha, cudaStream_t stream);
int beam_finalize_launch(const BeamState& s, int keep, long long* out_seq, int* out_len, float* out_p, float* out_raw, int* out_hist,
                         cudaStream_t stream);
int gather_logprob_rows_launch(const float* slab, long step_stride, long ld_slab, const int* hist, int nseq, int T, int V1, float* dst,
                               const float2* stats, long stats_stride, cudaStream_t stream, const long long* seqs = nullptr,
                               const DecodeEdits* ed = nullptr);

int layer_norm_launch(int rows, int D, const float* x, long ld_x, const float* a, const float* b, float eps, ActView out, cudaStream_t st);
int embed_pe_launch(int rows, int D, const int* tokens, const float* lut, const float* pe_row, float scale, ActView out, cudaStream_t st);
int enc_self_attention_launch(int B, int R, int heads, int dk, const float* q, const float* k, const float* v, long ld, const float* mask,
                              long ld_mask, ActView out, cudaStream_t st, int form = 0);
int dec_self_attention_launch(int rows, int heads, int dk, int t, const float* qkv, long ld_qkv, float* kcache, float* vcache, long step_stride,
                              long ld_c, const int* anc, long ld_anc, const long long* labels, long ld_lab, ActView out, cudaStream_t st, int form = 0);
int cross_attention_launch(int rows, int rpi, int heads, int dk, int R, const float* q, long ld_q, const float* kk, const float* vv, long ld_kv,
                           const float* mask, long ld_mask, ActView out, cudaStream_t st);

int glu_launch(int rows, int H, const float* t, long ld_t, const float* residual, long ld_res, ActView out, cudaStream_t st);
int masked_mean_launch(int B, int R, int H, const float* x, long ld_x, const float* mask, long ld_mask, ActView out, cudaStream_t st);

int gemm_generic_launch(int ta, int tb, int M, int N, int K, const float* A, long lda, const float* B, long ldb, float* C, long ldc, int accumulate,
                        const float* bias, cudaStream_t st);
int gemm_skinny_launch(int M, int N, int nseg, const float* const* A, const long* lda, const float* const* B, const long* ldb, const int* K, const int* tb,
                       float* C, long ldc, const float* bias, const float* row_bias, long ld_rb, int rpg, int accumulate, float* scratch,
                       size_t scratch_floats, int mode, cudaStream_t st);
int gemm_wgrad_launch(int M, int N, int K, const float* dY, long ld_dy, const float* X, long ld_x, float* G, long ld_g, int accumulate, int mode,
                      cudaStream_t st);
int colsum_launch(int rows, int cols, const float* x, long ld, float* out, int accumulate, cudaStream_t st);
struct Tf32Context;
Tf32Context* tf32_context_create();
void tf32_context_destroy(Tf32Context* c);
void tf32_context_new_step(Tf32Context* c);
long tf32_context_launches(const Tf32Context* c);
bool gemm_tf32_supported(int nseg, const float* const* X, const long* ldx, const float* const* W, const long* ldw, const int* K);
int gemm_tf32_launch(Tf32Context* ctx, int M, int N, int nseg, const float* const* X, const long* ldx, const float* const* W, const long* ldw, const int* K,
                     float* C, long ldc, const float* bias, const float* row_bias, long ld_rb, int rpg, int accumulate, cudaStream_t st);
const float* tf32_transposed(Tf32Context* ctx, const float* src, long ld_src, int rows, int cols, bool per_step, long* ld_dst, cudaStream_t st);
int dropout_apply_launch(float* x, int rows, int cols, long ld, unsigned long long seed, unsigned site, unsigned step, float p, cudaStream_t st);
int dropout_mask_launch(float* m, long n, unsigned long long seed, unsigned site, unsigned step, float p, cudaStream_t st);
int dropout_copy_launch(const float* x, long ld_x, float* y, long ld_y, int rows, int cols, unsigned long long seed, unsigned site, unsigned step, float p,
                        cudaStream_t st);
int embed_relu_dropout_launch(int rows, int E, const int* tokens, const float* emb, float* xt, unsigned long long seed, unsigned step, float p,
                              cudaStream_t st);
int scst_dlogits_launch(const float* logp, long ld_row, const long long* seq, const float* reward, const float* mask_sum, float upstream, int N, int T, int V1,
                        float* dl, cudaStream_t st, const float* row_coef = nullptr);
int scst_drop_worst_launch(const long long* seq, const float* row_loss, int N, int T, int keep, float upstream, float* row_msum, float* row_coef, float* loss,
                           cudaStream_t st);
int xe_loss_backward_launch(const float* logp, long ld_row, const long long* labels, long ld_l, const float* masks, long ld_m, int N, int steps, int Ls, int V1,
                            float smoothing, float upstream, float* mask_sum, float* item_loss, float* dl, float* loss, cudaStream_t st, int keep = 0,
                            float* row_loss = nullptr, float* row_msum = nullptr, float* row_coef = nullptr);
int logsoftmax_vjp_launch(const float* logp, const float* g, long ld_row, const long long* seq, int N, int T, int V1, float* dl, cudaStream_t st);
int lstm_cell_backward_launch(int rows, int H, const float* gates, const float* c_prev, const float* c_new, const float* dh, const float* dh_extra,
                              long ld_extra, unsigned drop_site, unsigned drop_step, unsigned long long seed, float p, float* dc_carry, float* dgates,
                              cudaStream_t st);
int maxout_cell_backward_launch(int rows, int H, const float* sums, const float* c_prev, const float* c_new, const float* dh, const float* dh_extra,
                                long ld_extra, unsigned drop_site, unsigned drop_step, unsigned long long seed, float p, float* dc_carry, float* dsums,
                                cudaStream_t st);
int attention_backward_launch(int n_images, int rpi, int R, int A, int H, const float* d_out, const float* alpha, const float* att_h, const float* p_att,
                              const float* att, const float* w, float* d_att_h, float* d_att, float* d_p_att, float* d_w, float* d_b, float* d_alpha_scratch,
                              cudaStream_t st);
int relu_dropout_backward_launch(long n, const float* x, const float* dy, float* dx, float scale, cudaStream_t st);
int embed_backward_launch(int rows, int E, const int* tokens, const float* xt, const float* dxt, long ld_dxt, float scale, float* d_emb, cudaStream_t st);
int embed_scatter_launch(int rows, int E, const int* tokens, const float* dxt, long ld_dxt, float* d_emb, cudaStream_t st);
int per_image_sum_launch(int steps, int rows, int rpi, int cols, const float* x, float* out, cudaStream_t st);
int add_strided_launch(float* a, const float* b, long ld_b, int rows, int cols, cudaStream_t st);

int ln_backward_launch(int rows, int D, const float* x, long ld_x, const float* a, const float* dy, long ld_dy, float eps, float* dx, long ld_dx, int accumulate,
                       float* stats, float* da, float* db, int accumulate_params, cudaStream_t st, const float* add1 = nullptr, long ld_a1 = 0,
                       const float* add2 = nullptr, long ld_a2 = 0);
int aoa_step_inputs_launch(int rows, int E, int H, int rpi, const int* tok_src, int* tok_dst, const float* emb, float* xt, const float* mean, long ld_mean,
                           const float* out_prev, float* x1c, unsigned long long seed, int step, float p_lm, float p_ctx, cudaStream_t st);
int glu_dropout_launch(int rows, int H, const float* t, long ld_t, float* out, long ld_o, float* outd, long ld_d, unsigned long long seed, int step, float p,
                       cudaStream_t st);
int glu_backward_fused_launch(int rows, int H, const float* t, long ld_t, const float* d_outd, long ld_dd, const float* dctx, float* dt, long ld_dt,
                              unsigned long long seed, int step, float p, cudaStream_t st);
int glu_backward_launch(int rows, int H, const float* t, long ld_t, const float* dy, long ld_dy, float* dt, long ld_dt, cudaStream_t st);
int dropout_salt_set_scst(unsigned long long salt, cudaStream_t st);
int dropout_salt_set_aoa(unsigned long long salt, cudaStream_t st);
int dropout_salt_set_tfm(unsigned long long salt, cudaStream_t st);
int dropout_salt_set_vocab(unsigned long long salt, cudaStream_t st);
int dropout_salt_set_attn(unsigned long long salt, cudaStream_t st);
inline int dropout_salt_set_all(unsigned long long salt, cudaStream_t st) {
    return dropout_salt_set_scst(salt, st) | dropout_salt_set_aoa(salt, st) | dropout_salt_set_tfm(salt, st) | dropout_salt_set_vocab(salt, st) |
// ... 69 lines not shown
```

imagecaptioning.pytorch_b200/csrc/pointwise.cu:

```cuda
#include "common.cuh"
#include "kernels.cuh"

namespace capb200 {

static int pw_blocks(long total) {
    long b = (total + 255) / 256;
    return (int)(b > sm_count() * 8 ? sm_count() * 8 : b);
}

namespace {

__device__ __forceinline__ float sigmoidf_(float x) { return fast_sigmoid(x); }

__device__ __forceinline__ void store_act(const ActView& o, long row, int col, float v) {
    o.f[row * o.ld + col] = v;
    if (o.hi != nullptr) {
        __half h, l;
        split_f32(v, h, l);
        o.hi[row * o.ld + col] = h;
        o.lo[row * o.ld + col] = l;
    }
}

__global__ void state_gather_embed_kernel(int rows, const int* __restrict__ tokens, const int* __restrict__ src_row,
                                          const float* __restrict__ emb, long ld_emb, int E, int relu, ActView xt,
                                          int H, int nstate, StateCopy sc0, StateCopy sc1) {
    const int r = blockIdx.x;
    if (r >= rows) return;
    const int tok = tokens[r];
    const float* e = emb + (long)tok * ld_emb;
    for (int c = threadIdx.x; c < E; c += blockDim.x) {
        float v = __ldg(e + c);
        if (relu) v = fmaxf(v, 0.f);
        store_act(xt, r, c, v);
    }
    const int src = src_row ? src_row[r] : r;
    const bool vec = (H & 3) == 0 && (sc0.ld_src & 3) == 0 && (sc0.dst.ld & 3) == 0 && (nstate < 2 || ((sc1.ld_src & 3) == 0 && (sc1.dst.ld & 3) == 0));
    if (vec) {
        for (int c4 = threadIdx.x; c4 < (H >> 2); c4 += blockDim.x) {
            float4 v0 = make_float4(0.f, 0.f, 0.f, 0.f), v1 = v0;
            if (src >= 0) {
                v0 = *reinterpret_cast<const float4*>(sc0.src + (long)src * sc0.ld_src + 4 * c4);
                if (nstate > 1) v1 = *reinterpret_cast<const float4*>(sc1.src + (long)src * sc1.ld_src + 4 * c4);
            }
            for (int s = 0; s < nstate; ++s) {
                const ActView& o = (s == 0) ? sc0.dst : sc1.dst;
                const float4 v = (s == 0) ? v0 : v1;
                *reinterpret_cast<float4*>(o.f + (long)r * o.ld + 4 * c4) = v;
                if (o.hi != nullptr) {
                    __align__(8) __half h[4];
                    __align__(8) __half l[4];
                    split_f32(v.x, h[0], l[0]); split_f32(v.y, h[1], l[1]); split_f32(v.z, h[2], l[2]); split_f32(v.w, h[3], l[3]);
                    *reinterpret_cast<uint2*>(o.hi + (long)r * o.ld + 4 * c4) = *reinterpret_cast<const uint2*>(h);
                    *reinterpret_cast<uint2*>(o.lo + (long)r * o.ld + 4 * c4) = *reinterpret_cast<const uint2*>(l);
                }
            }
        }
        return;
    }
    for (int s = 0; s < nstate; ++s) {
        const StateCopy& sc = (s == 0) ? sc0 : sc1;
        for (int c = threadIdx.x; c < H; c += blockDim.x) {
            const float v = (src < 0) ? 0.f : sc.src[(long)src * sc.ld_src + c];
            store_act(sc.dst, r, c, v);
        }
    }
}

__global__ void lstm_pointwise_kernel(int rows, int H, const float* __restrict__ gates, long ld_g, const int* __restrict__ src_row,
                                      const float* __restrict__ c_prev, long ld_cp, float* __restrict__ c_out, long ld_co, ActView h_out,
                                      const float* __restrict__ gather_bias, long ld_gb, const int* __restrict__ gather_idx) {
    const long total = (long)rows * H;
    for (long i = blockIdx.x * (long)blockDim.x + threadIdx.x; i < total; i += (long)gridDim.x * blockDim.x) {
        const int r = (int)(i / H), c = (int)(i % H);
        const float* g = gates + (long)r * ld_g;
        float gi = g[c], gf = g[H + c], gg = g[2 * H + c], go = g[3 * H + c];
        if (gather_bias != nullptr) {
            const float* gb = gather_bias + (long)gather_idx[r] * ld_gb;
            gi += __ldg(gb + c); gf += __ldg(gb + H + c); gg += __ldg(gb + 2 * H + c); go += __ldg(gb + 3 * H + c);
        }
        const int src = src_row ? src_row[r] : r;
        const float cp = (src < 0 || c_prev == nullptr) ? 0.f : c_prev[(long)src * ld_cp + c];
        const float cn = sigmoidf_(gf) * cp + sigmoidf_(gi) * fast_tanh(gg);
        const float hn = sigmoidf_(go) * fast_tanh(cn);
        c_out[(long)r * ld_co + c] = cn;
        store_act(h_out, r, c, hn);
    }
}

__global__ void __launch_bounds__(256) lstm_ln_kernel(int H, const float* __restrict__ gates, long ld_g, const float* __restrict__ c_prev, long ld_cp,
                                                      float* __restrict__ c_out, long ld_co, float* __restrict__ h_out, long ld_h, const float* __restrict__ ln_a,
                                                      const float* __restrict__ ln_b, float eps, float* __restrict__ ln_out, long ld_ln) {
    __shared__ float sh[8];
    const int r = blockIdx.x;
    const float* g = gates + (long)r * ld_g;
    float hv[8];
    float s = 0.f;
#pragma unroll
    for (int u = 0; u < 8; ++u) {
        const int c = threadIdx.x + 256 * u;
        hv[u] = 0.f;
        if (c < H) {
            const float gi = g[c], gf = g[H + c], gg = g[2 * H + c], go = g[3 * H + c];
            const float cp = c_prev == nullptr ? 0.f : c_prev[(long)r * ld_cp + c];
            const float cn = sigmoidf_(gf) * cp + sigmoidf_(gi) * fast_tanh(gg);
            const float hn = sigmoidf_(go) * fast_tanh(cn);
            c_out[(long)r * ld_co + c] = cn;
            h_out[(long)r * ld_h + c] = hn;
            hv[u] = hn;
            s += hn;
        }
    }
    auto bsum = [&](float v) {
#pragma unroll
        for (int o = 16; o > 0; o >>= 1) v += __shfl_xor_sync(0xffffffffu, v, o);
        __syncthreads();
        if ((threadIdx.x & 31) == 0) sh[threadIdx.x >> 5] = v;
        __syncthreads();
        return ((sh[0] + sh[1]) + (sh[2] + sh[3])) + ((sh[4] + sh[5]) + (sh[6] + sh[7]));
    };
    const float mean = bsum(s) / (float)H;
    float q = 0.f;
#pragma unroll
    for (int u = 0; u < 8; ++u) { const int c = threadIdx.x + 256 * u; if (c < H) { const float d = hv[u] - mean; q = fmaf(d, d, q); } }
    const float stdv = sqrtf(bsum(q) / (float)(H - 1));
    const float inv = 1.0f / (stdv + eps);
#pragma unroll
    for (int u = 0; u < 8; ++u) { const int c = threadIdx.x + 256 * u; if (c < H) ln_out[(long)r * ld_ln + c] = __ldg(ln_a + c) * (hv[u] - mean) * inv + __ldg(ln_b + c); }
}

__global__ void maxout_pointwise_kernel(int rows, int H, const float* __restrict__ sums, long ld_s, const int* __restrict__ src_row,
                                        const float* __restrict__ c_prev, long ld_cp, float* __restrict__ c_out, long ld_co, ActView h_out) {
    const long total = (long)rows * H;
    for (long i = blockIdx.x * (long)blockDim.x + threadIdx.x; i < total; i += (long)gridDim.x * blockDim.x) {
        const int r = (int)(i / H), c = (int)(i % H);
        const float* s = sums + (long)r * ld_s;
        const float gi = sigmoidf_(s[c]), gf = sigmoidf_(s[H + c]), go = sigmoidf_(s[2 * H + c]);
        const float gg = fmaxf(s[3 * H + c], s[4 * H + c]);
        const int src = src_row ? src_row[r] : r;
        const float cp = (src < 0 || c_prev == nullptr) ? 0.f : c_prev[(long)src * ld_cp + c];
// ... 229 lines not shown
```

imagecaptioning.pytorch_b200/csrc/vocab.cu:

```cuda
#include <cooperative_groups.h>
#include "common.cuh"
#include "kernels.cuh"

namespace cg = cooperative_groups;

namespace capb200 {

static __device__ unsigned long long g_vocab_seed_salt = 0ull;
int dropout_salt_set_vocab(unsigned long long salt, cudaStream_t st) {
    return cudaMemcpyToSymbolAsync(g_vocab_seed_salt, &salt, sizeof(salt), 0, cudaMemcpyHostToDevice, st) == cudaSuccess ? 0 : 1;
}

namespace {

constexpr int VT = 256;

template <int NT = VT>
__device__ __forceinline__ float block_max(float v, float* scratch) {
#pragma unroll
    for (int o = 16; o > 0; o >>= 1) v = fmaxf(v, __shfl_xor_sync(0xffffffffu, v, o));
    __syncthreads();
    if ((threadIdx.x & 31) == 0) scratch[threadIdx.x >> 5] = v;
    __syncthreads();
    float r = scratch[0];
#pragma unroll
    for (int w = 1; w < NT / 32; ++w) r = fmaxf(r, scratch[w]);
    return r;
}

template <int NT = VT>
__device__ __forceinline__ float block_sum(float v, float* scratch) {
#pragma unroll
    for (int o = 16; o > 0; o >>= 1) v += __shfl_xor_sync(0xffffffffu, v, o);
    __syncthreads();
    if ((threadIdx.x & 31) == 0) scratch[threadIdx.x >> 5] = v;
    __syncthreads();
    float r = 0.f;
#pragma unroll
    for (int w = 0; w < NT / 32; ++w) r += scratch[w];
    return r;
}

template <int NT = VT>
__device__ __forceinline__ void block_argmax(float v, int i, float* sval, int* sidx, float& out_v, int& out_i) {
#pragma unroll
    for (int o = 16; o > 0; o >>= 1) {
        const float ov = __shfl_xor_sync(0xffffffffu, v, o);
        const int oi = __shfl_xor_sync(0xffffffffu, i, o);
        if (ov > v || (ov == v && oi < i)) { v = ov; i = oi; }
    }
    __syncthreads();
    if ((threadIdx.x & 31) == 0) { sval[threadIdx.x >> 5] = v; sidx[threadIdx.x >> 5] = i; }
    __syncthreads();
    out_v = sval[0];
    out_i = sidx[0];
#pragma unroll
    for (int w = 1; w < NT / 32; ++w) {
        const float ov = sval[w];
        const int oi = sidx[w];
        if (ov > out_v || (ov == out_v && oi < out_i)) { out_v = ov; out_i = oi; }
    }
}

__device__ __forceinline__ uint32_t philox_first(uint32_t c0, uint32_t c1, uint32_t c2, uint32_t c3, uint32_t k0, uint32_t k1) {
#pragma unroll
    for (int r = 0; r < 10; ++r) {
        const uint32_t hi0 = __umulhi(0xD2511F53u, c0), lo0 = 0xD2511F53u * c0;
        const uint32_t hi1 = __umulhi(0xCD9E8D57u, c2), lo1 = 0xCD9E8D57u * c2;
        const uint32_t n0 = hi1 ^ c1 ^ k0, n1 = lo1, n2 = hi0 ^ c3 ^ k1, n3 = lo0;
        c0 = n0; c1 = n1; c2 = n2; c3 = n3;
        k0 += 0x9E3779B9u;
        k1 += 0xBB67AE85u;
    }
    return c0;
}

template <int KMAX, int NT, class Red>
__device__ __forceinline__ void vocab_step_row(const VocabStepArgs& a, int r, float* row, Red& red) {
    const int lo = red.lo, hi = red.hi, n = hi - lo;
    float* g = a.logits + (long)r * a.ld + lo;

    if (a.unfinished != nullptr && !a.first_step && a.unfinished[r] == 0) {
        for (int v = threadIdx.x; v < n; v += NT) g[v] = 0.f;
        if (red.lead && threadIdx.x == 0) {
            if (a.tokens_out) a.tokens_out[r] = 0;
// ... 249 lines not shown
    extern __shared__ float row[];
    __shared__ float s_red[NT / 32];
    __shared__ int s_idx[NT / 32];
    __shared__ ClusterSlots cs;
    cg::cluster_group cl = cg::this_cluster();
    const int rank = (int)cl.block_rank();
    const int lo = rank * S;
    RowInCluster<NT> red{s_red, s_idx, &cs, 0, lo, min(a.V1, lo + S), rank == 0};
    vocab_step_row<KMAX, NT>(a, blockIdx.x / cl.num_blocks(), row, red);
}

__global__ void __launch_bounds__(VT) vocab_stats_kernel(const VocabStepArgs a) {
    __shared__ float s_red[VT / 32];
    __shared__ int s_idx[VT / 32];
    const int r = blockIdx.x;
    const int V1 = a.V1;
    const float* g = a.logits + (long)r * a.ld;
    const bool vec = ((V1 & 3) == 0) && ((a.ld & 3) == 0) && ((reinterpret_cast<uintptr_t>(a.logits) & 15) == 0);
    float mx = -INFINITY;
    if (vec) {
        const float4* g4 = reinterpret_cast<const float4*>(g);
        for (int v = threadIdx.x; v < V1 / 4; v += VT) { const float4 x = g4[v]; mx = fmaxf(mx, fmaxf(fmaxf(x.x, x.y), fmaxf(x.z, x.w))); }
    } else {
        for (int v = threadIdx.x; v < V1; v += VT) mx = fmaxf(mx, g[v]);
    }
    mx = block_max(mx, s_red);
    float t0v = -INFINITY, t1v = -INFINITY;
    int t0i = 0x7fffffff, t1i = 0x7fffffff;
    float sum = 0.f;
    auto visit = [&](float x, int v) {
        sum += __expf(x - mx);
        if (x > t1v) {
            if (x > t0v) { t1v = t0v; t1i = t0i; t0v = x; t0i = v; }
            else { t1v = x; t1i = v; }
        }
    };
    if (vec) {
        const float4* g4 = reinterpret_cast<const float4*>(g);
        for (int v = threadIdx.x; v < V1 / 4; v += VT) {
            const float4 x = g4[v];
            visit(x.x, 4 * v); visit(x.y, 4 * v + 1); visit(x.z, 4 * v + 2); visit(x.w, 4 * v + 3);
        }
    } else {
        for (int v = threadIdx.x; v < V1; v += VT) visit(g[v], v);
    }
    sum = block_sum(sum, s_red);
    const float lsum = logf(sum);
    const float m2 = (mx - mx) - lsum, l2 = lsum;
    if (threadIdx.x == 0) a.stats[r] = make_float2(mx, lsum);
    int popped = 0;
    for (int k = 0; k < a.topk; ++k) {
        float ov;
        int oi;
        block_argmax(t0v, t0i, s_red, s_idx, ov, oi);
        if (t0i == oi && oi != 0x7fffffff) {
            const float lastv = t0v;
            const int lasti = t0i;
            t0v = t1v; t0i = t1i;
            t1v = -INFINITY; t1i = 0x7fffffff;
            if (++popped >= 2 && t0i == 0x7fffffff) {
                auto consider = [&](float x, int v) {
                    const bool after = (x < lastv) || (x == lastv && v > lasti);
                    if (after && (x > t0v || (x == t0v && v < t0i))) { t0v = x; t0i = v; }
                };
                if (vec) {
                    const float4* g4 = reinterpret_cast<const float4*>(g);
                    for (int v = threadIdx.x; v < V1 / 4; v += VT) {
                        const float4 x = g4[v];
                        consider(x.x, 4 * v); consider(x.y, 4 * v + 1); consider(x.z, 4 * v + 2); consider(x.w, 4 * v + 3);
                    }
                } else {
                    for (int v = threadIdx.x; v < V1; v += VT) consider(g[v], v);
                }
            }
        }
        if (threadIdx.x == 0) {
            const float lp = (ov - mx) - lsum;
            a.top_val[(long)r * a.topk + k] = a.row_twice(r) ? (lp - m2) - l2 : lp;
            a.top_idx[(long)r * a.topk + k] = oi;
        }
    }
}

__device__ __forceinline__ void online_raise(float& part, float& m, float& mL, float m4) {
    const float nL = m4 * 1.4426950408889634f;
    float sc;
    asm("ex2.approx.ftz.f32 %0, %1;" : "=f"(sc) : "f"(mL - nL));
    part = (m == -INFINITY) ? 0.f : part * sc;
    m = m4;
    mL = nL;
}
__device__ __forceinline__ float online_finish(float part, float m, float mL, float mx) {
    float sc;
    asm("ex2.approx.ftz.f32 %0, %1;" : "=f"(sc) : "f"(fmaf(-mx, 1.4426950408889634f, mL)));
    return (m == -INFINITY) ? 0.f : part * sc;
}

constexpr int VT2 = 128;
__device__ __forceinline__ float block_max4(float v, float* scratch) {
#pragma unroll
    for (int o = 16; o > 0; o >>= 1) v = fmaxf(v, __shfl_xor_sync(0xffffffffu, v, o));
    __syncthreads();
    if ((threadIdx.x & 31) == 0) scratch[threadIdx.x >> 5] = v;
    __syncthreads();
    return fmaxf(fmaxf(scratch[0], scratch[1]), fmaxf(scratch[2], scratch[3]));
}
__device__ __forceinline__ float block_sum4(float v, float* scratch) {
#pragma unroll
    for (int o = 16; o > 0; o >>= 1) v += __shfl_xor_sync(0xffffffffu, v, o);
    __syncthreads();
    if ((threadIdx.x & 31) == 0) scratch[threadIdx.x >> 5] = v;
    __syncthreads();
    return (scratch[0] + scratch[1]) + (scratch[2] + scratch[3]);
}
__device__ __forceinline__ void block_argmax4(float v, int i, float* sval, int* sidx, float& out_v, int& out_i) {
#pragma unroll
    for (int o = 16; o > 0; o >>= 1) {
        const float ov = __shfl_xor_sync(0xffffffffu, v, o);
        const int oi = __shfl_xor_sync(0xffffffffu, i, o);
        if (ov > v || (ov == v && oi < i)) { v = ov; i = oi; }
    }
    __syncthreads();
    if ((threadIdx.x & 31) == 0) { sval[threadIdx.x >> 5] = v; sidx[threadIdx.x >> 5] = i; }
    __syncthreads();
    out_v = sval[0];
    out_i = sidx[0];
#pragma unroll
    for (int w = 1; w < VT2 / 32; ++w) {
        const float ov = sval[w];
        const int oi = sidx[w];
        if (ov > out_v || (ov == out_v && oi < out_i)) { out_v = ov; out_i = oi; }
    }
}

__global__ void __launch_bounds__(VT2) vocab_stats_online128_kernel(const VocabStepArgs a) {
    __shared__ float s_red[VT2 / 32];
    __shared__ int s_idx[VT2 / 32];
    const int r = blockIdx.x;
    const int n4 = a.V1 >> 2;
    const float4* g4 = reinterpret_cast<const float4*>(a.logits + (long)r * a.ld);
    constexpr float kL2E = 1.4426950408889634f;
    float t0v = -INFINITY, t1v = -INFINITY;
    int t0i = 0x7fffffff, t1i = 0x7fffffff;
    float m = -INFINITY, mL = -INFINITY, part = 0.f;
    auto consume = [&](const float4 x, int v) {
        const float m4 = fmaxf(fmaxf(x.x, x.y), fmaxf(x.z, x.w));
        if (m4 > m) {
            online_raise(part, m, mL, m4);
        }
        float e0, e1, e2, e3;
        asm("ex2.approx.ftz.f32 %0, %1;" : "=f"(e0) : "f"(fmaf(x.x, kL2E, -mL)));
        asm("ex2.approx.ftz.f32 %0, %1;" : "=f"(e1) : "f"(fmaf(x.y, kL2E, -mL)));
        asm("ex2.approx.ftz.f32 %0, %1;" : "=f"(e2) : "f"(fmaf(x.z, kL2E, -mL)));
        asm("ex2.approx.ftz.f32 %0, %1;" : "=f"(e3) : "f"(fmaf(x.w, kL2E, -mL)));
        part += (e0 + e1) + (e2 + e3);
        if (m4 > t1v) {
            const float xs[4] = {x.x, x.y, x.z, x.w};
#pragma unroll
            for (int u = 0; u < 4; ++u) {
                if (xs[u] > t1v) {
                    if (xs[u] > t0v) { t1v = t0v; t1i = t0i; t0v = xs[u]; t0i = 4 * v + u; }
                    else { t1v = xs[u]; t1i = 4 * v + u; }
                }
            }
        }
    };
    int v = threadIdx.x;
    for (; v + 3 * VT2 < n4; v += 4 * VT2) {
        const float4 x0 = g4[v], x1 = g4[v + VT2], x2 = g4[v + 2 * VT2], x3 = g4[v + 3 * VT2];
        consume(x0, v); consume(x1, v + VT2); consume(x2, v + 2 * VT2); consume(x3, v + 3 * VT2);
    }
    for (; v < n4; v += VT2) consume(g4[v], v);
    const float mx = block_max4(m, s_red);
    float sum = online_finish(part, m, mL, mx);
    sum = block_sum4(sum, s_red);
    const float lsum = logf(sum);
    const float m2 = (mx - mx) - lsum, l2 = lsum;
    if (threadIdx.x == 0) a.stats[r] = make_float2(mx, lsum);
    int popped = 0;
    for (int k = 0; k < a.topk; ++k) {
        float ov;
        int oi;
        block_argmax4(t0v, t0i, s_red, s_idx, ov, oi);
        if (t0i == oi && oi != 0x7fffffff) {
            const float lastv = t0v;
            const int lasti = t0i;
            t0v = t1v; t0i = t1i;
            t1v = -INFINITY; t1i = 0x7fffffff;
            if (++popped >= 2 && t0i == 0x7fffffff) {
                auto consider = [&](float x, int w) {
                    const bool after = (x < lastv) || (x == lastv && w > lasti);
                    if (after && (x > t0v || (x == t0v && w < t0i))) { t0v = x; t0i = w; }
                };
                for (int w = threadIdx.x; w < n4; w += VT2) {
                    const float4 x = g4[w];
                    consider(x.x, 4 * w); consider(x.y, 4 * w + 1); consider(x.z, 4 * w + 2); consider(x.w, 4 * w + 3);
                }
            }
        }
        if (threadIdx.x == 0) {
            const float lp = (ov - mx) - lsum;
            a.top_val[(long)r * a.topk + k] = a.row_twice(r) ? (lp - m2) - l2 : lp;
            a.top_idx[(long)r * a.topk + k] = oi;
        }
    }
}

__global__ void __launch_bounds__(VT) ss_select_kernel(int V1, const float* __restrict__ prev_logp, long ld, const long long* __restrict__ labels,
                                                      long ld_labels, int col, unsigned long long seed, float prob, int* __restrict__ tok_out) {
    __shared__ float s_red[VT / 32];
    __shared__ int s_idx[VT / 32];
    const int r = blockIdx.x;
    seed ^= g_vocab_seed_salt;
    const uint32_t k0 = (uint32_t)seed ^ 0x6a09e667u, k1 = (uint32_t)(seed >> 32) ^ 0xbb67ae85u;
    const uint32_t ubits = philox_first(0xffffffffu, (uint32_t)r, (uint32_t)col, 6u, k0, k1);
    const float u_row = ((float)(ubits >> 9) + 0.5f) * (1.0f / 8388608.0f);
    if (!(u_row < prob)) {
        if (threadIdx.x == 0) tok_out[r] = (int)labels[(long)r * ld_labels + col];
        return;
    }
    const float* g = prev_logp + (long)r * ld;
    float bv = -INFINITY;
    int bi = 0x7fffffff;
    for (int v = threadIdx.x; v < V1; v += VT) {
        const uint32_t bits = philox_first((uint32_t)v, (uint32_t)r, (uint32_t)col, 6u, k0, k1);
        const float u = ((float)(bits >> 9) + 0.5f) * (1.0f / 8388608.0f);
        const float x = g[v] - logf(-logf(u));
        if (x > bv) { bv = x; bi = v; }
    }
    float ov;
    int tok;
    block_argmax(bv, bi, s_red, s_idx, ov, tok);
    if (threadIdx.x == 0) tok_out[r] = tok;
}

__global__ void mask_rows_kernel(ActView x, int R, int cols, const float* __restrict__ mask, long ld_mask) {
    const int row = blockIdx.x;
    const int img = row / R, r = row % R;
    if (mask[(long)img * ld_mask + r] != 0.f) return;
    for (int c = threadIdx.x; c < cols; c += blockDim.x) {
        x.f[(long)row * x.ld + c] = 0.f;
        if (x.hi) { x.hi[(long)row * x.ld + c] = __float2half(0.f); x.lo[(long)row * x.ld + c] = __float2half(0.f); }
    }
}

template <int KMAX>
int vocab_step_cluster_launch_k(const VocabStepArgs& a, cudaStream_t stream) {
    const int C = cdiv(a.V1, kRowSmem);
    const int S = cdiv(a.V1, C);
    static std::atomic<unsigned long long> configured{0};
    if (first_use_on_device(configured)) {
        CAPB_CHECK_CUDA(cudaFuncSetAttribute(vocab_step_cluster_kernel<KMAX, VTC>, cudaFuncAttributeMaxDynamicSharedMemorySize,
                                             (int)(sizeof(float) * kRowSmem)));
    }
    cudaLaunchConfig_t cfg = {};
    cfg.gridDim = dim3((unsigned)(a.rows * C));
    cfg.blockDim = dim3(VTC);
    cfg.dynamicSmemBytes = sizeof(float) * (size_t)S;
    cfg.stream = stream;
    cudaLaunchAttribute attr[1];
    attr[0].id = cudaLaunchAttributeClusterDimension;
    attr[0].val.clusterDim.x = (unsigned)C;
    attr[0].val.clusterDim.y = 1;
    attr[0].val.clusterDim.z = 1;
    cfg.attrs = attr;
    cfg.numAttrs = 1;
    CAPB_CHECK_CUDA(cudaLaunchKernelEx(&cfg, vocab_step_cluster_kernel<KMAX, VTC>, a, S));
    return 0;
}

int vocab_step_cluster_launch(const VocabStepArgs& a, cudaStream_t stream) {
    if (a.topk <= 2) return vocab_step_cluster_launch_k<2>(a, stream);
    if (a.topk <= 8) return vocab_step_cluster_launch_k<8>(a, stream);
    return vocab_step_cluster_launch_k<16>(a, stream);
}

}

int vocab_step_launch(const VocabStepArgs& a, cudaStream_t stream) {
    if (a.rows <= 0) return 0;
    CAPB_REQUIRE(a.topk <= 16, "beam size up to 16");
    if (a.stats != nullptr) {
        CAPB_REQUIRE(a.select == 0 && a.topk > 0, "stats mode is the beam-search epilogue");
        const bool vec = ((a.V1 & 3) == 0) && ((a.ld & 3) == 0) && ((reinterpret_cast<uintptr_t>(a.logits) & 15) == 0);
        if (vec) vocab_stats_online128_kernel<<<a.rows, VT2, 0, stream>>>(a);
        else vocab_stats_kernel<<<a.rows, VT, 0, stream>>>(a);
        CAPB_CHECK_CUDA(cudaGetLastError());
        return 0;
// ... 42 lines not shown
```

include/capb200.h:

```cpp
#ifndef CAPB200_H_
#define CAPB200_H_

#ifdef __cplusplus
extern "C" {
#endif

#define CAPB200_ABI_VERSION 1

#define CAPB200_MODE_SIMT_FP32 0
#define CAPB200_MODE_TC_F16X3 1
#define CAPB200_MODE_TC_F16X1 2
#define CAPB200_MODE_SKINNY_TF32X3 3
#define CAPB200_MODE_SKINNY_FP32 4
#define CAPB200_MODE_TF32X3_TC 5
#define CAPB200_MODE_TF32X3_TC_DGRAD 6
#define CAPB200_MODE_TF32X3_TC_WGRAD 7

#define CAPB200_MAX_SEQ_LENGTH 256

#define CAPB200_FAMILY_UPDOWN 0
#define CAPB200_FAMILY_NEWFC 1
#define CAPB200_FAMILY_ATT2IN2 2

typedef struct capb200_engine capb200_engine;
typedef struct capb200_cider_table capb200_cider_table;

const char* capb200_last_error(void);
int capb200_abi_version(void);
int capb200_range_status(int reset);


int capb200_linear(const float* x, long ldx, const float* w, long ldw, const float* b, float* y, long ldy, int M, int N, int K,
                   int relu, int mode, void* stream);

int capb200_bench_linear(const float* x, const float* w, const float* b, float* y, int M, int N, int K, int mode, int iters, float* ms_per_launch,
                         void* stream);

int capb200_gemm_tile_n(int M, int N);
int capb200_gemm_tile_m(int M, int N);

int capb200_lstm_cell(const float* x, int Kx, const float* h, const float* c, const float* w_ih, const float* w_hh, const float* b_ih,
                      const float* b_hh, float* h_out, float* c_out, int M, int H, int mode, void* stream);

int capb200_additive_attention(const float* att_h, const float* p_att, const float* att, const float* mask, const float* alpha_w,
                               const float* alpha_b, float* out, int n_images, int rows_per_image, int R, int A, int H, void* stream);

int capb200_log_softmax_topk(float* logits, long ld, int rows, int V1, int twice, int k, float* top_val, int* top_idx, void* stream);

int capb200_vocab_stats_topk(const float* logits, long ld, int rows, int V1, int twice, int k, float* stats, float* top_val, int* top_idx,
                             void* stream);

int capb200_vocab_select(float* logits, long ld, int rows, int V1, int select, float top, float temperature, unsigned long long seed,
                         unsigned long long step, int* unfinished, int first_step, int* tokens_out, float* picked_lp, void* stream);

typedef struct {
    int family;
    int vocab_size;
    int input_encoding_size;
    int rnn_size;
    int att_hid_size;
    int fc_feat_size;
    int att_feat_size;
    int seq_length;
    int numeric_mode;
} capb200_model_cfg;

typedef struct {
    const float* embed;
    const float *fc_embed_w, *fc_embed_b;
    const float *att_embed_w, *att_embed_b;
    const float *ctx2att_w, *ctx2att_b;
    const float *logit_w, *logit_b;
    const float *att_lstm_w_ih, *att_lstm_w_hh, *att_lstm_b_ih, *att_lstm_b_hh;
    const float *lang_lstm_w_ih, *lang_lstm_w_hh, *lang_lstm_b_ih, *lang_lstm_b_hh;
    const float *h2att_w, *h2att_b;
    const float *alpha_w, *alpha_b;
    const float *i2h_w, *i2h_b, *h2h_w, *h2h_b;
    const float *a2c_w, *a2c_b;
} capb200_weights;

capb200_engine* capb200_engine_create(const capb200_model_cfg* cfg);
void capb200_engine_destroy(capb200_engine* e);
int capb200_engine_bind_weights(capb200_engine* e, const capb200_weights* w, void* stream);

typedef struct {
    int decoding_constraint;
    int unk_col;
    int n_bad_endings;
    const int* bad_endings;
    int block_trigrams;
    int trigram_rows;
} capb200_decode_edits;

typedef struct {
    int beam_size;
    int sample_n;
    int penalty_kind;
    float penalty_alpha;
    float temperature;
    capb200_decode_edits edits;
} capb200_beam_opts;

int capb200_decode_beam(capb200_engine* e, const float* fc, const float* att, const float* mask, int B, int R, const capb200_beam_opts* opts,
                        long long* seq, float* seq_logprobs, long long* done_seq, int* done_len, float* done_p, float* done_raw, void* stream);
int capb200_beam_record_logprobs(capb200_engine* e, int image, int rank, float* dst, void* stream);

typedef struct {
    capb200_beam_opts base;
    int group_size;
    float diversity_lambda;
} capb200_diverse_opts;

int capb200_decode_beam_diverse(capb200_engine* e, const float* fc, const float* att, const float* mask, int B, int R, const capb200_diverse_opts* opts,
                                long long* seq, float* seq_logprobs, long long* done_seq, int* done_len, float* done_p, float* done_raw, void* stream);

#define CAPB200_SAMPLE_GREEDY 0
#define CAPB200_SAMPLE_MULTINOMIAL 1
#define CAPB200_SAMPLE_FORCED 2
#define CAPB200_SAMPLE_TEACHER 3
#define CAPB200_SAMPLE_TOPK 4
#define CAPB200_SAMPLE_TOPP 5
typedef struct {
    int sample_n;
    int method;
    float temperature;
    unsigned long long seed;
    int steps;
    float top;
    capb200_decode_edits edits;
} capb200_sample_opts;

int capb200_decode_sample(capb200_engine* e, const float* fc, const float* att, const float* mask, int B, int R, const capb200_sample_opts* opts,
                          const long long* tokens_in, long ld_tok, long long* seq, float* seq_logprobs, float* picked, void* stream);

long capb200_engine_launch_count(const capb200_engine* e);

int capb200_engine_set_profiling(capb200_engine* e, int enable);
int capb200_engine_read_profile(capb200_engine* e, int reset, double* ms, double* flops, long* calls, int n);

#define CAPB200_TFM_MAX_LAYERS 8
typedef struct capb200_tfm_engine capb200_tfm_engine;
typedef struct {
    int vocab_size, d_model, d_ff, heads, n_enc, n_dec, att_feat_size, seq_length, numeric_mode;
} capb200_tfm_cfg;
typedef struct { const float *q_w, *q_b, *k_w, *k_b, *v_w, *v_b, *o_w, *o_b; } capb200_mha_weights;
typedef struct {
    capb200_mha_weights self_attn;
    const float *w1_w, *w1_b, *w2_w, *w2_b;
    const float *ln0_a, *ln0_b, *ln1_a, *ln1_b;
} capb200_tfm_enc_layer;
typedef struct {
    capb200_mha_weights self_attn, src_attn;
    const float *w1_w, *w1_b, *w2_w, *w2_b;
    const float *ln0_a, *ln0_b, *ln1_a, *ln1_b, *ln2_a, *ln2_b;
} capb200_tfm_dec_layer;
typedef struct {
    const float *att_embed_w, *att_embed_b;
    capb200_tfm_enc_layer enc[CAPB200_TFM_MAX_LAYERS];
    const float *enc_norm_a, *enc_norm_b;
    capb200_tfm_dec_layer dec[CAPB200_TFM_MAX_LAYERS];
    const float *dec_norm_a, *dec_norm_b;
    const float *lut, *pe;
    const float *gen_w, *gen_b;
} capb200_tfm_weights;

capb200_tfm_engine* capb200_tfm_create(const capb200_tfm_cfg* cfg);
void capb200_tfm_destroy(capb200_tfm_engine* e);
int capb200_tfm_bind_weights(capb200_tfm_engine* e, const capb200_tfm_weights* w, void* stream);
int capb200_tfm_decode_beam(capb200_tfm_engine* e, const float* att, const float* mask, int B, int R, const capb200_beam_opts* opts, long long* seq,
                            float* seq_logprobs, long long* done_seq, int* done_len, float* done_p, float* done_raw, void* stream);
int capb200_tfm_beam_record_logprobs(capb200_tfm_engine* e, int image, int rank, float* dst, void* stream);
int capb200_tfm_decode_sample(capb200_tfm_engine* e, const float* att, const float* mask, int B, int R, const capb200_sample_opts* opts,
                              const long long* tokens_in, long ld_tok, long long* seq, float* seq_logprobs, float* picked, void* stream);
long capb200_tfm_launch_count(const capb200_tfm_engine* e);

#define CAPB200_AOA_REFINER_LAYERS 6
typedef struct capb200_aoa_engine capb200_aoa_engine;
typedef struct {
    int vocab_size, input_encoding_size, rnn_size, heads, att_feat_size, seq_length, numeric_mode;
} capb200_aoa_cfg;
typedef struct {
    const float *q_w, *q_b, *k_w, *k_b, *v_w, *v_b;
    const float *aoa_w, *aoa_b;
    const float *ln_a, *ln_b;
} capb200_aoa_refiner_layer;
typedef struct {
    const float* embed;
// ... 342 lines not shown
```

Measured before the change: 23970.

## Fuse vocab stats, beam selection and next-state gather into one beam-step kernel

Adds a per-image fused kernel that computes the online log-softmax and top-k for each live beam row in 128-thread groups, runs beam selection from shared memory, and gathers the next LSTM states. When it applies, the core step skips its own state gather. This removes two kernel launches per decode step and the global round trip for top-k values. In exchange there is one CTA per image with limited parallelism, and a named-barrier group scheme that adds complexity.

```diff
diff --git a/imagecaptioning.pytorch_b200/_lib.py b/imagecaptioning.pytorch_b200/_lib.py
--- a/imagecaptioning.pytorch_b200/_lib.py
+++ b/imagecaptioning.pytorch_b200/_lib.py
@@ -213,6 +213,8 @@
     'capb200_engine_bind_weights': (c_int, [c_void_p, POINTER(Weights), c_void_p]),
     'capb200_decode_beam': (c_int, [c_void_p, c_void_p, c_void_p, c_void_p, c_int, c_int, POINTER(BeamOpts), c_void_p, c_void_p, c_void_p, c_void_p,
                                     c_void_p, c_void_p, c_void_p]),
+    'capb200_decode_beam_form': (c_int, [c_int, c_void_p, c_void_p, c_void_p, c_void_p, c_int, c_int, POINTER(BeamOpts), c_void_p, c_void_p, c_void_p,
+                                         c_void_p, c_void_p, c_void_p, c_void_p]),
     'capb200_beam_record_logprobs': (c_int, [c_void_p, c_int, c_int, c_void_p, c_void_p]),
     'capb200_decode_beam_diverse': (c_int, [c_void_p, c_void_p, c_void_p, c_void_p, c_int, c_int, POINTER(DiverseOpts), c_void_p, c_void_p, c_void_p,
                                             c_void_p, c_void_p, c_void_p, c_void_p]),
diff --git a/imagecaptioning.pytorch_b200/csrc/beam.cu b/imagecaptioning.pytorch_b200/csrc/beam.cu
--- a/imagecaptioning.pytorch_b200/csrc/beam.cu
+++ b/imagecaptioning.pytorch_b200/csrc/beam.cu
@@ -1,6 +1,7 @@
 #include "../../include/capb200.h"
 #include "common.cuh"
 #include "kernels.cuh"
+#include "vocab_row.cuh"
 
 namespace capb200 {
 
@@ -14,24 +15,24 @@
     return p;
 }
 
-__device__ __forceinline__ void select_step(const BeamState& s, int img, int t, int live, int kl, int row0, int hist0, const float* __restrict__ top_val,
-                                            const int* __restrict__ top_idx, const int* pen, int n_pen, float lambda, int penalty_kind,
+template <int U = 8>
+__device__ __forceinline__ void select_step(const BeamState& s, int img, int t, int live, int kl, int row0, int hist0, const float* top_val,
+                                            const int* top_idx, const int* pen, int n_pen, float lambda, int penalty_kind,
                                             float penalty_alpha, double* __restrict__ done_p) {
     const int lane = threadIdx.x;
     const int b = s.beam, T = s.T;
     const int ncand = live * kl;
-    float cv[8];
-    int cf[8];
+    float cv[U];
+    int cf[U];
 #pragma unroll
-    for (int u = 0; u < 8; ++u) {
+    for (int u = 0; u < U; ++u) {
         const int c = lane + 32 * u;
         cv[u] = -INFINITY;
         cf[u] = 0x7fffffff;
         if (c < ncand) {
             const int pb = c / kl, k = c % kl;
-            const long row = (long)row0 + pb;
-            const int w = top_idx[row * kl + k];
-            float v = top_val[row * kl + k];
+            const int w = top_idx[pb * kl + k];
+            float v = top_val[pb * kl + k];
             int cnt = 0;
             for (int q = 0; q < n_pen; ++q) cnt += (pen[q] == w);
             if (cnt) v = __fsub_rn(v, __fmul_rn((float)cnt, lambda));
@@ -39,6 +40,7 @@
             cf[u] = pb * s.V1 + w;
         }
     }
+
     const int* seq_old = (t & 1) ? s.seq_b : s.seq_a;
     int* seq_new = (t & 1) ? s.seq_a : s.seq_b;
     const int* hist_old = (t & 1) ? s.hist_b : s.hist_a;
@@ -50,7 +52,7 @@
         float bv = -INFINITY;
         int bf = 0x7fffffff, bu = -1;
 #pragma unroll
-        for (int u = 0; u < 8; ++u)
+        for (int u = 0; u < U; ++u)
             if (cv[u] > bv || (cv[u] == bv && cf[u] < bf)) { bv = cv[u]; bf = cf[u]; bu = u; }
         float wv = bv;
         int wf = bf;
@@ -62,7 +64,7 @@
         }
         if (bu >= 0 && bf == wf && bv == wv) {
 #pragma unroll
-            for (int u = 0; u < 8; ++u) if (u == bu) { cv[u] = -INFINITY; cf[u] = 0x7fffffff; }
+            for (int u = 0; u < U; ++u) if (u == bu) { cv[u] = -INFINITY; cf[u] = 0x7fffffff; }
         }
         if (lane == j) { my_v = wv; my_f = wf; }
     }
@@ -76,6 +78,7 @@
     const int slot = cnt0 + __popc(em & ((1u << lane) - 1u));
     if (has) { sh_parent[lane] = parent; sh_word[lane] = word; sh_slot[lane] = ended ? slot : -1; }
     __syncwarp();
+#pragma unroll 1
     for (int idx = lane; idx < b * t; idx += 32) {
         const int j = idx / t, q = idx - j * t;
         const long dst = ((long)img * b + j) * T, src = ((long)img * b + sh_parent[j]) * T;
@@ -83,6 +86,7 @@
         hist_new[dst + q] = hist_old[src + q];
     }
     if (em != 0u) {
+#pragma unroll 1
         for (int idx = lane; idx < b * (t + 1); idx += 32) {
             const int j = idx / (t + 1), q = idx - j * (t + 1);
             if (sh_slot[j] < 0) continue;
@@ -114,7 +118,33 @@
                                                        const int* __restrict__ top_idx, int penalty_kind, float penalty_alpha,
                                                        double* __restrict__ done_p) {
     const int img = blockIdx.x;
-    select_step(s, img, t, live, s.beam, img * live, img * live, top_val, top_idx, nullptr, 0, 0.f, penalty_kind, penalty_alpha, done_p);
+    const long row0 = (long)img * live;
+    select_step(s, img, t, live, s.beam, (int)row0, (int)row0, top_val + row0 * s.beam, top_idx + row0 * s.beam, nullptr, 0, 0.f, penalty_kind,
+                penalty_alpha, done_p);
+}
+
+constexpr int kStepGroups = 8;
+template <int U>
+__global__ void __maxnreg__(U <= 2 ? 48 : 64) beam_search_step_kernel(BeamState s, const VocabStepArgs a, int t, int live, int penalty_kind, float penalty_alpha,
+                                                        double* __restrict__ done_p, NextStateGather next) {
+    __shared__ float s_red[kStepGroups][VT2 / 32];
+    __shared__ int s_ridx[kStepGroups][VT2 / 32];
+    __shared__ float s_val[MAXB * MAXB];
+    __shared__ int s_idx[MAXB * MAXB];
+    const int img = blockIdx.x, g = threadIdx.x / VT2, ng = blockDim.x / VT2;
+    const int b = s.beam, row0 = img * live;
+    for (int j = g; j < live; j += ng)
+        stats_online128_row(a, row0 + j, threadIdx.x % VT2, GroupBarrier{1 + g}, s_red[g], s_ridx[g], s_val + j * b, s_idx + j * b);
+    __syncthreads();
+    if (threadIdx.x < 32) select_step<U>(s, img, t, live, b, row0, row0, s_val, s_idx, nullptr, 0, 0.f, penalty_kind, penalty_alpha, done_p);
+    if (t == s.T - 1) return;
+    __syncthreads();
+    const int n4 = next.H >> 2;
+    for (int i = threadIdx.x; i < b * n4; i += blockDim.x) {
+        const int j = i / n4, c4 = i - j * n4;
+        const long r = (long)img * b + j;
+        copy_states4(r, s.src_row[r], c4, 2, next.s0, next.s1);
+    }
 }
 
 __global__ void __launch_bounds__(32) diverse_beam_step_kernel(BeamState s, int G, int t, int k, const float* __restrict__ top_val,
@@ -136,8 +166,8 @@
         }
         __syncwarp();
         const int vimg = i * G + g;
-        select_step(s, vimg, lt, lt == 0 ? 1 : b, k, vimg * b, g * rows_total + vimg * b, top_val, top_idx, sh_pen, n_pen, lambda, penalty_kind,
-                    penalty_alpha, done_p);
+        select_step(s, vimg, lt, lt == 0 ? 1 : b, k, vimg * b, g * rows_total + vimg * b, top_val + (long)vimg * b * k, top_idx + (long)vimg * b * k,
+                    sh_pen, n_pen, lambda, penalty_kind, penalty_alpha, done_p);
     }
 }
 
@@ -320,6 +350,29 @@
     return 0;
 }
 
+bool beam_search_step_applies(const VocabStepArgs& a, const NextStateGather& next) {
+    auto al16 = [](const void* p) { return (reinterpret_cast<uintptr_t>(p) & 15) == 0; };
+    auto al8 = [](const void* p) { return (reinterpret_cast<uintptr_t>(p) & 7) == 0; };
+    auto state_ok = [&](const StateCopy& c) {
+        return c.src != nullptr && c.dst.f != nullptr && (c.ld_src & 3) == 0 && (c.dst.ld & 3) == 0 && al16(c.src) && al16(c.dst.f) &&
+               ((c.dst.hi == nullptr) == (c.dst.lo == nullptr)) && (c.dst.hi == nullptr || (al8(c.dst.hi) && al8(c.dst.lo)));
+    };
+    return (a.V1 & 3) == 0 && (a.ld & 3) == 0 && al16(a.logits) && next.H > 0 && (next.H & 3) == 0 && state_ok(next.s0) && state_ok(next.s1);
+}
+
+int beam_search_step_launch(const BeamState& s, const VocabStepArgs& a, int t, int live, int penalty_kind, float penalty_alpha,
+                            const NextStateGather& next, cudaStream_t stream) {
+    CAPB_REQUIRE(s.beam >= 1 && s.beam <= MAXB, "beam size 1..16");
+    CAPB_REQUIRE(s.beam * s.T <= MAXB * CAPB200_MAX_SEQ_LENGTH, "beam*T record capacity (16 x CAPB200_MAX_SEQ_LENGTH)");
+    CAPB_REQUIRE(a.topk == s.beam && a.stats != nullptr && a.rows == s.B * live && live >= 1 && live <= s.beam, "fused beam step arguments");
+    CAPB_REQUIRE(beam_search_step_applies(a, next), "the fused beam step needs 16-byte aligned logit and state rows (V + 1 and H multiples of 4)");
+    const int threads = min(live, kStepGroups) * VT2;
+    if (s.beam <= 8) beam_search_step_kernel<2><<<s.B, threads, 0, stream>>>(s, a, t, live, penalty_kind, penalty_alpha, s.done_p, next);
+    else beam_search_step_kernel<8><<<s.B, threads, 0, stream>>>(s, a, t, live, penalty_kind, penalty_alpha, s.done_p, next);
+    CAPB_CHECK_CUDA(cudaGetLastError());
+    return 0;
+}
+
 int diverse_beam_step_launch(const BeamState& s, int G, int t, int k, const float* top_val, const int* top_idx, float lambda, int rows_total,
                              int penalty_kind, float penalty_alpha, cudaStream_t stream) {
     CAPB_REQUIRE(G >= 2 && s.beam >= 1 && G * s.beam <= MAXB, "group_size * beams per group must be in 2..16");
diff --git a/imagecaptioning.pytorch_b200/csrc/engine.cu b/imagecaptioning.pytorch_b200/csrc/engine.cu
--- a/imagecaptioning.pytorch_b200/csrc/engine.cu
+++ b/imagecaptioning.pytorch_b200/csrc/engine.cu
@@ -324,7 +324,7 @@
 }
 
 int core_step(capb200_engine* e, int rows, int rpi, const int* tokens, const int* src_row, float* logits, long ld_logits, int n_images, int R,
-              const float* mask, cudaStream_t st) {
+              const float* mask, cudaStream_t st, bool states_gathered = false) {
     const int H = e->H, E = e->E, A = e->A, V1 = e->V1;
     const capb200_weights& w = e->w;
     if (e->cfg.family == CAPB200_FAMILY_UPDOWN) {
@@ -332,8 +332,11 @@
         s0.src = e->h0_out.v.f; s0.ld_src = e->h0_out.v.ld; s0.dst = e->h0_in.v;
         s1.src = e->h1_out.v.f; s1.ld_src = e->h1_out.v.ld; s1.dst = e->h1_in.v;
         const bool xg = e->use_xgate;
-        e->launches++;
-        if (state_gather_embed_launch(rows, tokens, src_row, w.embed, E, xg ? 0 : E, 1, e->xt.v, H, 2, s0, s1, st)) return 1;
+        CAPB_REQUIRE(!states_gathered || xg, "the fused beam step gathers the states only; the word embedding needs the separate gather");
+        if (!states_gathered) {
+            e->launches++;
+            if (state_gather_embed_launch(rows, tokens, src_row, w.embed, E, xg ? 0 : E, 1, e->xt.v, H, 2, s0, s1, st)) return 1;
+        }
         const int cur = e->core_cur, nxt = cur ^ 1;
         {
             GemmProblem g;
@@ -516,7 +519,7 @@
 
 int lstm_decode_core(capb200_engine* e, int rows, int rpi, const int* tokens, const int* src_row, float* logits, long ld, int B, int R,
                      const float* mask, cudaStream_t st) {
-    return core_step(e, rows, rpi, tokens, src_row, logits, ld, B, R, mask, st);
+    return core_step(e, rows, rpi, tokens, src_row, logits, ld, B, R, mask, st, e->d.states_gathered);
 }
 
 }
@@ -720,8 +723,8 @@
     return 0;
 }
 
-int capb200_decode_beam(capb200_engine* e, const float* fc, const float* att, const float* mask, int B, int R, const capb200_beam_opts* opts,
-                        long long* seq, float* seq_logprobs, long long* done_seq, int* done_len, float* done_p, float* done_raw, void* stream) {
+static int decode_beam(capb200_engine* e, const float* fc, const float* att, const float* mask, int B, int R, const capb200_beam_opts* opts,
+                       long long* seq, float* seq_logprobs, long long* done_seq, int* done_len, float* done_p, float* done_raw, void* stream, int form) {
     if (check_ready(e)) return 1;
     cudaStream_t st = static_cast<cudaStream_t>(stream);
     CAPB_REQUIRE(opts != nullptr && (fc != nullptr || e->cfg.family == CAPB200_FAMILY_ATT2IN2) && seq != nullptr, "null argument");
@@ -739,9 +742,27 @@
     auto core = [&](int nrows, int live, const int* tokens, const int* src_row, int , float* logits, long ld) {
         return lstm_decode_core(e, nrows, live, tokens, src_row, logits, ld, B, R, mask, st);
     };
+    NextStateGather next;
+    const bool gather = e->cfg.family == CAPB200_FAMILY_UPDOWN && e->use_xgate;
+    if (gather) {
+        next.s0.src = e->h0_out.v.f; next.s0.ld_src = e->h0_out.v.ld; next.s0.dst = e->h0_in.v;
+        next.s1.src = e->h1_out.v.f; next.s1.ld_src = e->h1_out.v.ld; next.s1.dst = e->h1_in.v;
+        next.H = e->H;
+    }
     return beam_decode_driver(e->d, V1, T, B, beam, keep, opts->penalty_kind, opts->penalty_alpha, seq, seq_logprobs, done_seq, done_len, done_p,
                               done_raw, core, &e->launches, st, e->profiling ? 0ull : loop_graph_key(e->ws, e->wblock, mask, R, (int)e->cfg.family),
-                              to_edits(opts->edits), opts->temperature);
+                              to_edits(opts->edits), opts->temperature, gather ? &next : nullptr, form);
+}
+
+int capb200_decode_beam(capb200_engine* e, const float* fc, const float* att, const float* mask, int B, int R, const capb200_beam_opts* opts,
+                        long long* seq, float* seq_logprobs, long long* done_seq, int* done_len, float* done_p, float* done_raw, void* stream) {
+    return decode_beam(e, fc, att, mask, B, R, opts, seq, seq_logprobs, done_seq, done_len, done_p, done_raw, stream, 0);
+}
+
+int capb200_decode_beam_form(int form, capb200_engine* e, const float* fc, const float* att, const float* mask, int B, int R,
+                             const capb200_beam_opts* opts, long long* seq, float* seq_logprobs, long long* done_seq, int* done_len, float* done_p,
+                             float* done_raw, void* stream) {
+    return decode_beam(e, fc, att, mask, B, R, opts, seq, seq_logprobs, done_seq, done_len, done_p, done_raw, stream, form);
 }
 
 int capb200_decode_beam_diverse(capb200_engine* e, const float* fc, const float* att, const float* mask, int B, int R, const capb200_diverse_opts* opts,
diff --git a/imagecaptioning.pytorch_b200/csrc/engine_common.cuh b/imagecaptioning.pytorch_b200/csrc/engine_common.cuh
--- a/imagecaptioning.pytorch_b200/csrc/engine_common.cuh
+++ b/imagecaptioning.pytorch_b200/csrc/engine_common.cuh
@@ -113,6 +113,7 @@
     unsigned long long loop_key[8] = {0, 0, 0, 0, 0, 0, 0, 0}, seen_key[8] = {0, 0, 0, 0, 0, 0, 0, 0};
     long loop_launches = 0;
     bool graph_broken = false;
+    bool states_gathered = false;
 
     void release() {
         if (loop_exec) cudaGraphExecDestroy(loop_exec);
@@ -234,12 +235,14 @@
 template <class CoreFn>
 int beam_decode_driver(DecodeBuffers& d, int V1, int T, int B, int beam, int keep, int penalty_kind, float penalty_alpha, long long* seq,
                        float* seq_logprobs, long long* done_seq, int* done_len, float* done_p, float* done_raw, CoreFn core, long* launches,
-                       cudaStream_t st, unsigned long long graph_key = 0, const DecodeEdits& ed = DecodeEdits(), float temperature = 1.0f) {
+                       cudaStream_t st, unsigned long long graph_key = 0, const DecodeEdits& ed = DecodeEdits(), float temperature = 1.0f,
+                       const NextStateGather* next = nullptr, int form = 0) {
     const int rows = B * beam;
     const bool edits = ed.any();
     const int k_in = beam + ed.kinds();
     CAPB_REQUIRE(!ed.trigrams, "block_trigrams applies to _sample only (AttModel.py:306)");
     CAPB_REQUIRE(k_in <= 16, "beam_size + number of active decode edits (decoding_constraint, remove_bad_endings, UNK suppression) must be <= 16");
+    CAPB_REQUIRE(form >= 0 && form <= 2, "beam step form must be 0 (automatic), 1 (separate kernels) or 2 (fused)");
     if (temperature == 0.f) temperature = 1.0f;
     CAPB_REQUIRE(temperature > 0.f, "temperature must be positive");
     if (grow_buffer(reinterpret_cast<void**>(&d.slab), &d.slab_bytes, (size_t)T * rows * V1 * sizeof(float), st)) return 1;
@@ -248,6 +251,14 @@
     d.last_beam = beam;
     BeamState s = d.bs;
     s.B = B; s.beam = beam; s.T = T; s.V1 = V1;
+    bool fused = false;
+    if (form != 1 && next != nullptr && !edits && temperature == 1.0f) {
+        VocabStepArgs probe;
+        probe.V1 = V1; probe.ld = V1; probe.logits = d.slab;
+        fused = beam_search_step_applies(probe, *next);
+    }
+    CAPB_REQUIRE(form != 2 || fused, "the fused beam step needs the engine's state descriptor, no decode edits, temperature 1 and 16-byte aligned "
+                                     "logit and state rows (V + 1 and H multiples of 4)");
     auto run_loop = [&]() -> int {
         CAPB_NVTX("capb200 beam loop (T steps: core, vocab stats, beam step)");
         CAPB_CHECK_CUDA(cudaMemsetAsync(s.sums, 0, sizeof(float) * B * beam, st));
@@ -257,7 +268,10 @@
             const int live = (t == 0) ? 1 : beam;
             const int nrows = B * live;
             float* logits = d.slab + (long)t * d.slab_step_stride;
-            if (core(nrows, live, d.tokens, t == 0 ? d.neg1 : d.src_row, t, logits, (long)V1)) return 1;
+            d.states_gathered = fused && t > 0;
+            const int rc = core(nrows, live, d.tokens, t == 0 ? d.neg1 : d.src_row, t, logits, (long)V1);
+            d.states_gathered = false;
+            if (rc) return 1;
             if (t > 0 && temperature != 1.0f) {
                 if (scale_rows_launch(logits, V1, nrows, V1, 1.0f / temperature, st)) return 1;
                 *launches += 1;
@@ -267,6 +281,11 @@
             va.twice = (t > 0) ? 1 : 0;
             va.topk = edits ? k_in : beam; va.top_val = d.top_val; va.top_idx = d.top_idx;
             va.stats = d.slab_stats + (long)t * rows;
+            if (fused) {
+                if (beam_search_step_launch(s, va, t, live, penalty_kind, penalty_alpha, *next, st)) return 1;
+                *launches += 1;
+                continue;
+            }
             if (vocab_step_launch(va, st)) return 1;
             const float* tv = d.top_val;
             const int* ti = d.top_idx;
@@ -285,6 +304,7 @@
     memcpy(&key[6], &penalty_alpha, sizeof(float));
     memcpy(reinterpret_cast<char*>(&key[6]) + 4, &temperature, sizeof(float));
     key[5] ^= ((unsigned long long)(ed.constraint & 1) << 8) ^ ((unsigned long long)(unsigned)(ed.unk_col + 1) << 16) ^ ((unsigned long long)ed.n_bad << 48);
+    key[5] ^= (unsigned long long)fused << 9;
     key[0] ^= (unsigned long long)reinterpret_cast<uintptr_t>(ed.bad) * 0x9E3779B97F4A7C15ull;
     d.last_edits = ed;
     d.last_stats = d.slab_stats;
diff --git a/imagecaptioning.pytorch_b200/csrc/kernels.cuh b/imagecaptioning.pytorch_b200/csrc/kernels.cuh
--- a/imagecaptioning.pytorch_b200/csrc/kernels.cuh
+++ b/imagecaptioning.pytorch_b200/csrc/kernels.cuh
@@ -15,6 +15,26 @@
     long ld_src = 0;
     ActView dst;
 };
+
+__device__ __forceinline__ void copy_states4(long r, int src, int c4, int nstate, const StateCopy& sc0, const StateCopy& sc1) {
+    float4 v0 = make_float4(0.f, 0.f, 0.f, 0.f), v1 = v0;
+    if (src >= 0) {
+        v0 = *reinterpret_cast<const float4*>(sc0.src + (long)src * sc0.ld_src + 4 * c4);
+        if (nstate > 1) v1 = *reinterpret_cast<const float4*>(sc1.src + (long)src * sc1.ld_src + 4 * c4);
+    }
+    for (int s = 0; s < nstate; ++s) {
+        const ActView& o = (s == 0) ? sc0.dst : sc1.dst;
+        const float4 v = (s == 0) ? v0 : v1;
+        *reinterpret_cast<float4*>(o.f + r * o.ld + 4 * c4) = v;
+        if (o.hi != nullptr) {
+            __align__(8) __half h[4];
+            __align__(8) __half l[4];
+            split_f32(v.x, h[0], l[0]); split_f32(v.y, h[1], l[1]); split_f32(v.z, h[2], l[2]); split_f32(v.w, h[3], l[3]);
+            *reinterpret_cast<uint2*>(o.hi + r * o.ld + 4 * c4) = *reinterpret_cast<const uint2*>(h);
+            *reinterpret_cast<uint2*>(o.lo + r * o.ld + 4 * c4) = *reinterpret_cast<const uint2*>(l);
+        }
+    }
+}
 
 int state_gather_embed_launch(int rows, const int* tokens, const int* src_row, const float* emb, long ld_emb, int E, int relu,
                               ActView xt, int H, int nstate, StateCopy sc0, StateCopy sc1, cudaStream_t stream);
@@ -99,6 +119,13 @@
 };
 int beam_step_launch(const BeamState& s, int t, int live, const float* top_val, const int* top_idx, int penalty_kind, float penalty_alpha,
                      cudaStream_t stream);
+struct NextStateGather {
+    StateCopy s0, s1;
+    int H = 0;
+};
+bool beam_search_step_applies(const VocabStepArgs& a, const NextStateGather& next);
+int beam_search_step_launch(const BeamState& s, const VocabStepArgs& a, int t, int live, int penalty_kind, float penalty_alpha,
+                            const NextStateGather& next, cudaStream_t stream);
 int diverse_beam_step_launch(const BeamState& s, int G, int t, int k, const float* top_val, const int* top_idx, float lambda, int rows_total,
                              int penalty_kind, float penalty_alpha, cudaStream_t stream);
 int beam_finalize_launch(const BeamState& s, int keep, long long* out_seq, int* out_len, float* out_p, float* out_raw, int* out_hist,
diff --git a/imagecaptioning.pytorch_b200/csrc/pointwise.cu b/imagecaptioning.pytorch_b200/csrc/pointwise.cu
--- a/imagecaptioning.pytorch_b200/csrc/pointwise.cu
+++ b/imagecaptioning.pytorch_b200/csrc/pointwise.cu
@@ -37,25 +37,7 @@
     const int src = src_row ? src_row[r] : r;
     const bool vec = (H & 3) == 0 && (sc0.ld_src & 3) == 0 && (sc0.dst.ld & 3) == 0 && (nstate < 2 || ((sc1.ld_src & 3) == 0 && (sc1.dst.ld & 3) == 0));
     if (vec) {
-        for (int c4 = threadIdx.x; c4 < (H >> 2); c4 += blockDim.x) {
-            float4 v0 = make_float4(0.f, 0.f, 0.f, 0.f), v1 = v0;
-            if (src >= 0) {
-                v0 = *reinterpret_cast<const float4*>(sc0.src + (long)src * sc0.ld_src + 4 * c4);
-                if (nstate > 1) v1 = *reinterpret_cast<const float4*>(sc1.src + (long)src * sc1.ld_src + 4 * c4);
-            }
-            for (int s = 0; s < nstate; ++s) {
-                const ActView& o = (s == 0) ? sc0.dst : sc1.dst;
-                const float4 v = (s == 0) ? v0 : v1;
-                *reinterpret_cast<float4*>(o.f + (long)r * o.ld + 4 * c4) = v;
-                if (o.hi != nullptr) {
-                    __align__(8) __half h[4];
-                    __align__(8) __half l[4];
-                    split_f32(v.x, h[0], l[0]); split_f32(v.y, h[1], l[1]); split_f32(v.z, h[2], l[2]); split_f32(v.w, h[3], l[3]);
-                    *reinterpret_cast<uint2*>(o.hi + (long)r * o.ld + 4 * c4) = *reinterpret_cast<const uint2*>(h);
-                    *reinterpret_cast<uint2*>(o.lo + (long)r * o.ld + 4 * c4) = *reinterpret_cast<const uint2*>(l);
-                }
-            }
-        }
+        for (int c4 = threadIdx.x; c4 < (H >> 2); c4 += blockDim.x) copy_states4(r, src, c4, nstate, sc0, sc1);
         return;
     }
     for (int s = 0; s < nstate; ++s) {
diff --git a/imagecaptioning.pytorch_b200/csrc/vocab.cu b/imagecaptioning.pytorch_b200/csrc/vocab.cu
--- a/imagecaptioning.pytorch_b200/csrc/vocab.cu
+++ b/imagecaptioning.pytorch_b200/csrc/vocab.cu
@@ -1,6 +1,7 @@
 #include <cooperative_groups.h>
 #include "common.cuh"
 #include "kernels.cuh"
+#include "vocab_row.cuh"
 
 namespace cg = cooperative_groups;
 
@@ -416,128 +417,11 @@
     }
 }
 
-__device__ __forceinline__ void online_raise(float& part, float& m, float& mL, float m4) {
-    const float nL = m4 * 1.4426950408889634f;
-    float sc;
-    asm("ex2.approx.ftz.f32 %0, %1;" : "=f"(sc) : "f"(mL - nL));
-    part = (m == -INFINITY) ? 0.f : part * sc;
-    m = m4;
-    mL = nL;
-}
-__device__ __forceinline__ float online_finish(float part, float m, float mL, float mx) {
-    float sc;
-    asm("ex2.approx.ftz.f32 %0, %1;" : "=f"(sc) : "f"(fmaf(-mx, 1.4426950408889634f, mL)));
-    return (m == -INFINITY) ? 0.f : part * sc;
-}
-
-constexpr int VT2 = 128;
-__device__ __forceinline__ float block_max4(float v, float* scratch) {
-#pragma unroll
-    for (int o = 16; o > 0; o >>= 1) v = fmaxf(v, __shfl_xor_sync(0xffffffffu, v, o));
-    __syncthreads();
-    if ((threadIdx.x & 31) == 0) scratch[threadIdx.x >> 5] = v;
-    __syncthreads();
-    return fmaxf(fmaxf(scratch[0], scratch[1]), fmaxf(scratch[2], scratch[3]));
-}
-__device__ __forceinline__ float block_sum4(float v, float* scratch) {
-#pragma unroll
-    for (int o = 16; o > 0; o >>= 1) v += __shfl_xor_sync(0xffffffffu, v, o);
-    __syncthreads();
-    if ((threadIdx.x & 31) == 0) scratch[threadIdx.x >> 5] = v;
-    __syncthreads();
-    return (scratch[0] + scratch[1]) + (scratch[2] + scratch[3]);
-}
-__device__ __forceinline__ void block_argmax4(float v, int i, float* sval, int* sidx, float& out_v, int& out_i) {
-#pragma unroll
-    for (int o = 16; o > 0; o >>= 1) {
-        const float ov = __shfl_xor_sync(0xffffffffu, v, o);
-        const int oi = __shfl_xor_sync(0xffffffffu, i, o);
-        if (ov > v || (ov == v && oi < i)) { v = ov; i = oi; }
-    }
-    __syncthreads();
-    if ((threadIdx.x & 31) == 0) { sval[threadIdx.x >> 5] = v; sidx[threadIdx.x >> 5] = i; }
-    __syncthreads();
-    out_v = sval[0];
-    out_i = sidx[0];
-#pragma unroll
-    for (int w = 1; w < VT2 / 32; ++w) {
-        const float ov = sval[w];
-        const int oi = sidx[w];
-        if (ov > out_v || (ov == out_v && oi < out_i)) { out_v = ov; out_i = oi; }
-    }
-}
-
 __global__ void __launch_bounds__(VT2) vocab_stats_online128_kernel(const VocabStepArgs a) {
     __shared__ float s_red[VT2 / 32];
     __shared__ int s_idx[VT2 / 32];
     const int r = blockIdx.x;
-    const int n4 = a.V1 >> 2;
-    const float4* g4 = reinterpret_cast<const float4*>(a.logits + (long)r * a.ld);
-    constexpr float kL2E = 1.4426950408889634f;
-    float t0v = -INFINITY, t1v = -INFINITY;
-    int t0i = 0x7fffffff, t1i = 0x7fffffff;
-    float m = -INFINITY, mL = -INFINITY, part = 0.f;
-    auto consume = [&](const float4 x, int v) {
-        const float m4 = fmaxf(fmaxf(x.x, x.y), fmaxf(x.z, x.w));
-        if (m4 > m) {
-            online_raise(part, m, mL, m4);
-        }
-        float e0, e1, e2, e3;
-        asm("ex2.approx.ftz.f32 %0, %1;" : "=f"(e0) : "f"(fmaf(x.x, kL2E, -mL)));
-        asm("ex2.approx.ftz.f32 %0, %1;" : "=f"(e1) : "f"(fmaf(x.y, kL2E, -mL)));
-        asm("ex2.approx.ftz.f32 %0, %1;" : "=f"(e2) : "f"(fmaf(x.z, kL2E, -mL)));
-        asm("ex2.approx.ftz.f32 %0, %1;" : "=f"(e3) : "f"(fmaf(x.w, kL2E, -mL)));
-        part += (e0 + e1) + (e2 + e3);
-        if (m4 > t1v) {
-            const float xs[4] = {x.x, x.y, x.z, x.w};
-#pragma unroll
-            for (int u = 0; u < 4; ++u) {
-                if (xs[u] > t1v) {
-                    if (xs[u] > t0v) { t1v = t0v; t1i = t0i; t0v = xs[u]; t0i = 4 * v + u; }
-                    else { t1v = xs[u]; t1i = 4 * v + u; }
-                }
-            }
-        }
-    };
-    int v = threadIdx.x;
-    for (; v + 3 * VT2 < n4; v += 4 * VT2) {
-        const float4 x0 = g4[v], x1 = g4[v + VT2], x2 = g4[v + 2 * VT2], x3 = g4[v + 3 * VT2];
-        consume(x0, v); consume(x1, v + VT2); consume(x2, v + 2 * VT2); consume(x3, v + 3 * VT2);
-    }
-    for (; v < n4; v += VT2) consume(g4[v], v);
-    const float mx = block_max4(m, s_red);
-    float sum = online_finish(part, m, mL, mx);
-    sum = block_sum4(sum, s_red);
-    const float lsum = logf(sum);
-    const float m2 = (mx - mx) - lsum, l2 = lsum;
-    if (threadIdx.x == 0) a.stats[r] = make_float2(mx, lsum);
-    int popped = 0;
-    for (int k = 0; k < a.topk; ++k) {
-        float ov;
-        int oi;
-        block_argmax4(t0v, t0i, s_red, s_idx, ov, oi);
-        if (t0i == oi && oi != 0x7fffffff) {
-            const float lastv = t0v;
-            const int lasti = t0i;
-            t0v = t1v; t0i = t1i;
-            t1v = -INFINITY; t1i = 0x7fffffff;
-            if (++popped >= 2 && t0i == 0x7fffffff) {
-                auto consider = [&](float x, int w) {
-                    const bool after = (x < lastv) || (x == lastv && w > lasti);
-                    if (after && (x > t0v || (x == t0v && w < t0i))) { t0v = x; t0i = w; }
-                };
-                for (int w = threadIdx.x; w < n4; w += VT2) {
-                    const float4 x = g4[w];
-                    consider(x.x, 4 * w); consider(x.y, 4 * w + 1); consider(x.z, 4 * w + 2); consider(x.w, 4 * w + 3);
-                }
-            }
-        }
-        if (threadIdx.x == 0) {
-            const float lp = (ov - mx) - lsum;
-            a.top_val[(long)r * a.topk + k] = a.row_twice(r) ? (lp - m2) - l2 : lp;
-            a.top_idx[(long)r * a.topk + k] = oi;
-        }
-    }
+    stats_online128_row(a, r, threadIdx.x, CtaBarrier{}, s_red, s_idx, a.top_val + (long)r * a.topk, a.top_idx + (long)r * a.topk);
 }
 
 __global__ void __launch_bounds__(VT) ss_select_kernel(int V1, const float* __restrict__ prev_logp, long ld, const long long* __restrict__ labels,
diff --git a/imagecaptioning.pytorch_b200/csrc/vocab_row.cuh b/imagecaptioning.pytorch_b200/csrc/vocab_row.cuh
--- /dev/null
+++ b/imagecaptioning.pytorch_b200/csrc/vocab_row.cuh
@@ -0,0 +1,142 @@
+#pragma once
+#include "common.cuh"
+#include "kernels.cuh"
+
+namespace capb200 {
+
+__device__ __forceinline__ void online_raise(float& part, float& m, float& mL, float m4) {
+    const float nL = m4 * 1.4426950408889634f;
+    float sc;
+    asm("ex2.approx.ftz.f32 %0, %1;" : "=f"(sc) : "f"(mL - nL));
+    part = (m == -INFINITY) ? 0.f : part * sc;
+    m = m4;
+    mL = nL;
+}
+__device__ __forceinline__ float online_finish(float part, float m, float mL, float mx) {
+    float sc;
+    asm("ex2.approx.ftz.f32 %0, %1;" : "=f"(sc) : "f"(fmaf(-mx, 1.4426950408889634f, mL)));
+    return (m == -INFINITY) ? 0.f : part * sc;
+}
+
+constexpr int VT2 = 128;
+
+struct CtaBarrier {
+    __device__ __forceinline__ void operator()() const { __syncthreads(); }
+};
+struct GroupBarrier {
+    int id;
+    __device__ __forceinline__ void operator()() const { asm volatile("bar.sync %0, %1;" ::"r"(id), "r"(VT2) : "memory"); }
+};
+
+template <class Bar>
+__device__ __forceinline__ float block_max4(float v, float* scratch, int tid, Bar bar) {
+#pragma unroll
+    for (int o = 16; o > 0; o >>= 1) v = fmaxf(v, __shfl_xor_sync(0xffffffffu, v, o));
+    bar();
+    if ((tid & 31) == 0) scratch[tid >> 5] = v;
+    bar();
+    return fmaxf(fmaxf(scratch[0], scratch[1]), fmaxf(scratch[2], scratch[3]));
+}
+template <class Bar>
+__device__ __forceinline__ float block_sum4(float v, float* scratch, int tid, Bar bar) {
+#pragma unroll
+    for (int o = 16; o > 0; o >>= 1) v += __shfl_xor_sync(0xffffffffu, v, o);
+    bar();
+    if ((tid & 31) == 0) scratch[tid >> 5] = v;
+    bar();
+    return (scratch[0] + scratch[1]) + (scratch[2] + scratch[3]);
+}
+template <class Bar>
+__device__ __forceinline__ void block_argmax4(float v, int i, float* sval, int* sidx, int tid, Bar bar, float& out_v, int& out_i) {
+#pragma unroll
+    for (int o = 16; o > 0; o >>= 1) {
+        const float ov = __shfl_xor_sync(0xffffffffu, v, o);
+        const int oi = __shfl_xor_sync(0xffffffffu, i, o);
+        if (ov > v || (ov == v && oi < i)) { v = ov; i = oi; }
+    }
+    bar();
+    if ((tid & 31) == 0) { sval[tid >> 5] = v; sidx[tid >> 5] = i; }
+    bar();
+    out_v = sval[0];
+    out_i = sidx[0];
+#pragma unroll
+    for (int w = 1; w < VT2 / 32; ++w) {
+        const float ov = sval[w];
+        const int oi = sidx[w];
+        if (ov > out_v || (ov == out_v && oi < out_i)) { out_v = ov; out_i = oi; }
+    }
+}
+
+template <class Bar>
+__device__ __forceinline__ void stats_online128_row(const VocabStepArgs& a, int r, int tid, Bar bar, float* s_red, int* s_idx, float* top_val,
+                                                    int* top_idx) {
+    const int n4 = a.V1 >> 2;
+    const float4* g4 = reinterpret_cast<const float4*>(a.logits + (long)r * a.ld);
+    constexpr float kL2E = 1.4426950408889634f;
+    float t0v = -INFINITY, t1v = -INFINITY;
+    int t0i = 0x7fffffff, t1i = 0x7fffffff;
+    float m = -INFINITY, mL = -INFINITY, part = 0.f;
+    auto consume = [&](const float4 x, int v) {
+        const float m4 = fmaxf(fmaxf(x.x, x.y), fmaxf(x.z, x.w));
+        if (m4 > m) {
+            online_raise(part, m, mL, m4);
+        }
+        float e0, e1, e2, e3;
+        asm("ex2.approx.ftz.f32 %0, %1;" : "=f"(e0) : "f"(fmaf(x.x, kL2E, -mL)));
+        asm("ex2.approx.ftz.f32 %0, %1;" : "=f"(e1) : "f"(fmaf(x.y, kL2E, -mL)));
+        asm("ex2.approx.ftz.f32 %0, %1;" : "=f"(e2) : "f"(fmaf(x.z, kL2E, -mL)));
+        asm("ex2.approx.ftz.f32 %0, %1;" : "=f"(e3) : "f"(fmaf(x.w, kL2E, -mL)));
+        part += (e0 + e1) + (e2 + e3);
+        if (m4 > t1v) {
+            const float xs[4] = {x.x, x.y, x.z, x.w};
+#pragma unroll
+            for (int u = 0; u < 4; ++u) {
+                if (xs[u] > t1v) {
+                    if (xs[u] > t0v) { t1v = t0v; t1i = t0i; t0v = xs[u]; t0i = 4 * v + u; }
+                    else { t1v = xs[u]; t1i = 4 * v + u; }
+                }
+            }
+        }
+    };
+    int v = tid;
+    for (; v + 3 * VT2 < n4; v += 4 * VT2) {
+        const float4 x0 = g4[v], x1 = g4[v + VT2], x2 = g4[v + 2 * VT2], x3 = g4[v + 3 * VT2];
+        consume(x0, v); consume(x1, v + VT2); consume(x2, v + 2 * VT2); consume(x3, v + 3 * VT2);
+    }
+    for (; v < n4; v += VT2) consume(g4[v], v);
+    const float mx = block_max4(m, s_red, tid, bar);
+    float sum = online_finish(part, m, mL, mx);
+    sum = block_sum4(sum, s_red, tid, bar);
+    const float lsum = logf(sum);
+    const float m2 = (mx - mx) - lsum, l2 = lsum;
+    if (tid == 0) a.stats[r] = make_float2(mx, lsum);
+    int popped = 0;
+    for (int k = 0; k < a.topk; ++k) {
+        float ov;
+        int oi;
+        block_argmax4(t0v, t0i, s_red, s_idx, tid, bar, ov, oi);
+        if (t0i == oi && oi != 0x7fffffff) {
+            const float lastv = t0v;
+            const int lasti = t0i;
+            t0v = t1v; t0i = t1i;
+            t1v = -INFINITY; t1i = 0x7fffffff;
+            if (++popped >= 2 && t0i == 0x7fffffff) {
+                auto consider = [&](float x, int w) {
+                    const bool after = (x < lastv) || (x == lastv && w > lasti);
+                    if (after && (x > t0v || (x == t0v && w < t0i))) { t0v = x; t0i = w; }
+                };
+                for (int w = tid; w < n4; w += VT2) {
+                    const float4 x = g4[w];
+                    consider(x.x, 4 * w); consider(x.y, 4 * w + 1); consider(x.z, 4 * w + 2); consider(x.w, 4 * w + 3);
+                }
+            }
+        }
+        if (tid == 0) {
+            const float lp = (ov - mx) - lsum;
+            top_val[k] = a.row_twice(r) ? (lp - m2) - l2 : lp;
+            top_idx[k] = oi;
+        }
+    }
+}
+
+}
diff --git a/include/capb200.h b/include/capb200.h
--- a/include/capb200.h
+++ b/include/capb200.h
@@ -103,6 +103,9 @@
 
 int capb200_decode_beam(capb200_engine* e, const float* fc, const float* att, const float* mask, int B, int R, const capb200_beam_opts* opts,
                         long long* seq, float* seq_logprobs, long long* done_seq, int* done_len, float* done_p, float* done_raw, void* stream);
+int capb200_decode_beam_form(int form, capb200_engine* e, const float* fc, const float* att, const float* mask, int B, int R,
+                             const capb200_beam_opts* opts, long long* seq, float* seq_logprobs, long long* done_seq, int* done_len, float* done_p,
+                             float* done_raw, void* stream);
 int capb200_beam_record_logprobs(capb200_engine* e, int image, int rank, float* dst, void* stream);
 
 typedef struct {
```

Result: faster. 24770, median of 6 (+3.3%).
